# youssefg7/dl-sound-classification

Hardware: AMD Instinct MI355X
Metric: training clips/sec (EnvNet-v2, ESC-50 shape) (higher is better)
Workload: dtype bf16; 1 GPU; EnvNet-v2 train step (BC-mix, fwd, soft-CE, bwd, clip, Adam), ESC-50 shape; global_batch=256, per_gpu_batch=256, clip_samples=220500, parallelism=dp1, model=envnet_v2

## Files before the change

### dl-sound-classification_amd/csrc/common.h

```cpp
#pragma once
#include <hip/hip_runtime.h>
#include <stdint.h>
#include <stdio.h>
#include <string.h>
#include <math.h>

#include "../../include/miaudio.h"

typedef __bf16 bf16;
typedef __bf16 bf16x8 __attribute__((ext_vector_type(8)));
typedef __bf16 bf16x4 __attribute__((ext_vector_type(4)));
typedef __bf16 bf16x2 __attribute__((ext_vector_type(2)));
typedef float f32x2_cvt __attribute__((ext_vector_type(2)));
typedef unsigned u32x4 __attribute__((ext_vector_type(4)));

__device__ __forceinline__ uint32_t pk_bf16(float lo, float hi) {
  return __builtin_bit_cast(uint32_t, __builtin_convertvector(f32x2_cvt{lo, hi}, bf16x2));
}
typedef float f32x16 __attribute__((ext_vector_type(16)));
typedef float f32x4 __attribute__((ext_vector_type(4)));
typedef short s16x4 __attribute__((ext_vector_type(4)));

#define MIA_LDS __attribute__((address_space(3)))

namespace mia {
void set_error(const char* fmt, ...);
int fail(int code, const char* fmt, ...);
int cu_count();
}

#define MIA_CHECK_ARG(cond, ...)                       \
  do {                                                 \
    if (!(cond)) return mia::fail(-22, __VA_ARGS__);   \
  } while (0)

#define MIA_LAUNCH_CHECK(what)                                                   \
  do {                                                                           \
    hipError_t e__ = hipGetLastError();                                          \
    if (e__ != hipSuccess)                                                       \
      return mia::fail(-(int)e__, "%s: launch failed: %s", what, hipGetErrorString(e__)); \
  } while (0)

static inline hipStream_t as_stream(mia_stream_t s) { return reinterpret_cast<hipStream_t>(s); }
static inline int64_t cdiv(int64_t a, int64_t b) { return (a + b - 1) / b; }
static inline bool aligned16(const void* p) { return (reinterpret_cast<uintptr_t>(p) & 15) == 0; }

__device__ __forceinline__ float bf2f(bf16 x) { return (float)x; }
__device__ __forceinline__ bf16 f2bf(float x) { return (bf16)x; }

__device__ __forceinline__ void wave_sync() {
  __builtin_amdgcn_fence(__ATOMIC_ACQ_REL, "wavefront");
  __builtin_amdgcn_wave_barrier();
}

template <typename T> __device__ __forceinline__ float to_f(T x);
template <> __device__ __forceinline__ float to_f<float>(float x) { return x; }
template <> __device__ __forceinline__ float to_f<bf16>(bf16 x) { return (float)x; }
template <typename T> __device__ __forceinline__ T from_f(float x);
template <> __device__ __forceinline__ float from_f<float>(float x) { return x; }
template <> __device__ __forceinline__ bf16 from_f<bf16>(float x) { return (bf16)x; }

__device__ __forceinline__ float ld_elem(const void* p, int dtype, int64_t i) {
  return dtype == MIA_F32 ? ((const float*)p)[i] : (float)((const bf16*)p)[i];
}
__device__ __forceinline__ void st_elem(void* p, int dtype, int64_t i, float v) {
  if (dtype == MIA_F32) ((float*)p)[i] = v;
  else ((bf16*)p)[i] = (bf16)v;
}

__device__ __forceinline__ float wave_sum(float v) {
#pragma unroll
  for (int o = 32; o > 0; o >>= 1) v += __shfl_xor(v, o, 64);
  return v;
}
__device__ __forceinline__ void lds_barrier() { asm volatile("s_waitcnt lgkmcnt(0)\n\ts_barrier" ::: "memory"); }

__device__ __forceinline__ double wave_sum_d(double v) {
#pragma unroll
  for (int o = 32; o > 0; o >>= 1) v += __shfl_xor(v, o, 64);
  return v;
}
__device__ __forceinline__ double block_sum_strided(const float* __restrict__ p, int n, int64_t stride) {
  __shared__ double red_bss[256];
  double s = 0.0;
  for (int k = threadIdx.x; k < n; k += 256) s += (double)p[(int64_t)k * stride];
  red_bss[threadIdx.x] = s;
  __syncthreads();
  for (int w = 128; w > 0; w >>= 1) {
    if ((int)threadIdx.x < w) red_bss[threadIdx.x] += red_bss[threadIdx.x + w];
    __syncthreads();
  }
  const double r = red_bss[0];
  __syncthreads();
  return r;
}

constexpr int COLSUM_SLICES = 16;
inline int64_t colsum_part2_bytes(int cols) { return (int64_t)COLSUM_SLICES * cols * 8; }
static __global__ __launch_bounds__(256) void colsum_pass1_kernel(const float* __restrict__ p, int64_t rows, int cols,
                                                                  int64_t ld, double* __restrict__ part2) {
  __shared__ double red_cp[4][64];
  const int l = threadIdx.x & 63, g = threadIdx.x >> 6;
  const int c = blockIdx.x * 64 + l;
  const int64_t per = (rows + gridDim.y - 1) / gridDim.y;
  const int64_t r0 = (int64_t)blockIdx.y * per, r1 = r0 + per < rows ? r0 + per : rows;
  double s = 0.0;
  if (c < cols) {
#pragma unroll 8
    for (int64_t r = r0 + g; r < r1; r += 4) s += (double)p[r * ld + c];
  }
  red_cp[g][l] = s;
  __syncthreads();
  if (g == 0 && c < cols)
    part2[(int64_t)blockIdx.y * cols + c] = ((red_cp[0][l] + red_cp[1][l]) + red_cp[2][l]) + red_cp[3][l];
}
inline void colsum_pass1(const float* p, int64_t rows, int cols, int64_t ld, double* part2, hipStream_t s) {
  colsum_pass1_kernel<<<dim3((unsigned)((cols + 63) / 64), COLSUM_SLICES), 256, 0, s>>>(p, rows, cols, ld, part2);
}
__device__ __forceinline__ double colsum_slices(const double* __restrict__ part2, int cols, int c) {
  double v = 0.0;
#pragma unroll
  for (int y = 0; y < COLSUM_SLICES; ++y) v += part2[(int64_t)y * cols + c];
  return v;
}

__device__ __forceinline__ int mx_exponent(float amax) {
  const int be = (int)((__float_as_uint(amax) >> 23) & 0xff);
  const int e = be == 0 ? -127 : be - 127 - 8;
// ... 95 lines not shown
```

### dl-sound-classification_amd/csrc/conv3w.hip

```cpp
#include <cstdlib>

#include "bn_math.h"
#include "channel_partials.h"

namespace {

typedef unsigned u32x2 __attribute__((ext_vector_type(2)));
typedef short s16x8 __attribute__((ext_vector_type(8)));

struct W3Args {
  const bf16* x;
  const bf16* dy;
  float* part;
  int n, h, wd, oh, ow, nseg;
  const bf16* ya;
  bf16* dyo;
  float* bpart;
  const float *gamma, *scale, *shift, *mean, *invstd, *dgamma, *dbeta;
  int64_t P;
};

__device__ __forceinline__ bf16x8 tr_frag(const char* p0, int stride) {
  const s16x4 lo = __builtin_amdgcn_ds_read_tr16_b64_v4i16((MIA_LDS s16x4*)(p0));
  const s16x4 hi = __builtin_amdgcn_ds_read_tr16_b64_v4i16((MIA_LDS s16x4*)(p0 + 4 * stride));
// ... 87 lines not shown
    const int qq = lane + 64 * s;
    const int px = seg * 32 + (qq >> 2);
    const u32x4 v = {o[0], o[1], o[2], o[3]};
    *reinterpret_cast<u32x4*>(g.dyo + (((int64_t)b * g.oh + oy) * g.ow + px) * 32 + (qq & 3) * 8) = v;
    return v;
  };
  auto run = [&](const Raw& R, int it) __attribute__((always_inline)) {
    u32x4 dv[2] = {R.d[0], R.d[1]};
    if constexpr (BN) {
      dv[0] = bn_chunk(R, 0, it);
      dv[1] = bn_chunk(R, 1, it);
    }
    wave_sync();
    if (lane < 40) {
      const int l = lane;
      const int r = l / 5, q = l % 5;
      const uint32_t d[6] = {R.v[0][0], R.v[0][1], R.v[1][0], R.v[1][1], R.v[2][0], R.v[2][1]};
#pragma unroll
      for (int c = 0; c < 4; ++c) {
        uint32_t o[4];
#pragma unroll
        for (int i = 0; i < 4; ++i) {
          const int e = c + 2 * i;
          o[i] = (e & 1) ? ((d[e >> 1] >> 16) | (d[(e >> 1) + 1] << 16)) : d[e >> 1];
        }
        *reinterpret_cast<u32x4*>(sg + c * CPYB + r * ROWB + 16 * q) = u32x4{o[0], o[1], o[2], o[3]};
      }
    }
#pragma unroll
    for (int s = 0; s < 2; ++s) {
      const int qq = lane + 64 * s;
      *reinterpret_cast<u32x4*>(dt + (qq >> 2) * 64 + (qq & 3) * 16) = dv[s];
    }
    wave_sync();
    const int kx = n & 7, cp = kx & 3;
#pragma unroll
    for (int ks = 0; ks < 2; ++ks) {
      const int kr = ks * 16 + 8 * (gq >> 1) + (i16 >> 2);
      const int c4 = 16 * (gq & 1) + 4 * (i16 & 3);
      const bf16x8 fa = tr_frag(dt + kr * 64 + c4 * 2, 64);
#pragma unroll
      for (int nt = 0; nt < 2; ++nt) {
        const int ky = 4 * nt + (n >> 3);
        const char* src = sg + cp * CPYB + ky * ROWB + 2 * (16 * ks + 8 * h + (kx & 4));
        const u32x2 p0 = *reinterpret_cast<const u32x2*>(src);
        const u32x2 p1 = *reinterpret_cast<const u32x2*>(src + 8);
        const u32x4 f = {p0[0], p0[1], p1[0], p1[1]};
        acc[nt] = __builtin_amdgcn_mfma_f32_32x32x16_bf16(fa, __builtin_bit_cast(bf16x8, f), acc[nt], 0, 0, 0);
      }
    }
  };

  int it = gw;
  if (it < items) {
    Raw ra = load(it), rb;
    for (;;) {
      rb = load(it + nw);
      run(ra, it);
      it += nw;
      if (it >= items) break;
      ra = load(it + nw);
      run(rb, it);
      it += nw;
      if (it >= items) break;
    }
  }
  float* dst = g.part + (int64_t)gw * 2048;
#pragma unroll
  for (int nt = 0; nt < 2; ++nt)
#pragma unroll
    for (int r = 0; r < 16; ++r) {
      const int co = (r & 3) + 8 * (r >> 2) + 4 * h;
      dst[co * 64 + nt * 32 + n] = acc[nt][r];
    }
  if constexpr (BN) {
#pragma unroll
    for (int i = 0; i < 8; ++i)
#pragma unroll
      for (int m = 4; m < 64; m <<= 1) bs1[i] += __shfl_xor(bs1[i], m, 64);
    if (lane < 4) {
#pragma unroll
      for (int i = 0; i < 8; ++i) g.bpart[(int64_t)gw * 32 + lane * 8 + i] = bs1[i];
    }
  }
}

constexpr int C3_G = 64;
__global__ __launch_bounds__(256) void conv3_wgrad_reduce1_kernel(const float* __restrict__ part, int nslab,
                                                                  double* __restrict__ tmp) {
  const int e = blockIdx.x * 256 + threadIdx.x, gi = blockIdx.y;
  const int per = (nslab + C3_G - 1) / C3_G;
  const int w0 = gi * per, w1 = min(nslab, w0 + per);
  double s = 0.0;
  for (int w = w0; w < w1; ++w) s += (double)part[(int64_t)w * 2048 + e];
  tmp[gi * 2048 + e] = s;
}
__global__ __launch_bounds__(256) void conv3_wgrad_reduce1x16_kernel(const float* __restrict__ part, int nslab,
                                                                     double* __restrict__ tmp) {
  const int e = blockIdx.x * 256 + threadIdx.x, gi = blockIdx.y;
  const int per = (nslab + C3_G - 1) / C3_G;
  const int w0 = gi * per, w1 = min(nslab, w0 + per);
  const float* p = part + e;
  double s = 0.0;
  int w = w0;
  for (; w + 16 <= w1; w += 16) {
    float v[16];
#pragma unroll
    for (int u = 0; u < 16; ++u) v[u] = p[(int64_t)(w + u) * 2048];
#pragma unroll
    for (int u = 0; u < 16; ++u) s += (double)v[u];
  }
  for (; w < w1; ++w) s += (double)p[(int64_t)w * 2048];
  tmp[gi * 2048 + e] = s;
}
void conv3_wgrad_reduce1(const float* part, int nslab, double* tmp, hipStream_t s) {
  const char* v1 = getenv("MIA_REDUCE_V1");
  if (v1 && v1[0] == '1') conv3_wgrad_reduce1_kernel<<<dim3(8, C3_G), 256, 0, s>>>(part, nslab, tmp);
  else conv3_wgrad_reduce1x16_kernel<<<dim3(8, C3_G), 256, 0, s>>>(part, nslab, tmp);
}
__global__ __launch_bounds__(256) void conv3_wgrad_reduce2_kernel(const double* __restrict__ tmp, float* __restrict__ dw) {
  const int e = blockIdx.x * 256 + threadIdx.x;
  double s = 0.0;
#pragma unroll 8
  for (int g = 0; g < C3_G; ++g) s += tmp[g * 2048 + e];
  dw[e] = (float)s;
}

}

extern "C" int mia_conv3_wgrad(const void* x, const void* dy, float* dw, float* part, int32_t nwaves, int32_t n,
                               int32_t h, int32_t wd, mia_stream_t stream) {
  MIA_CHECK_ARG(x && dy && dw && part && n > 0 && h >= 8 && wd >= 8, "conv3_wgrad: bad arguments");
  MIA_CHECK_ARG(nwaves > 0 && nwaves % 4 == 0, "conv3_wgrad: nwaves must be a positive multiple of 4");
  MIA_CHECK_ARG(wd % 4 == 0, "conv3_wgrad: image width must be a multiple of 4 (8-byte row alignment)");
  MIA_CHECK_ARG((reinterpret_cast<uintptr_t>(dy) & 15) == 0 && (reinterpret_cast<uintptr_t>(x) & 7) == 0,
                "conv3_wgrad: dy must be 16-byte and x 8-byte aligned");
  W3Args a{reinterpret_cast<const bf16*>(x), reinterpret_cast<const bf16*>(dy), part, n, h, wd, h - 7, wd - 7,
           (int)cdiv(wd - 7, 32)};
  MIA_CHECK_ARG((int64_t)n * a.oh * a.nseg < (1ll << 31), "conv3_wgrad: too many items");
  hipStream_t s = as_stream(stream);
  conv3_wgrad_kernel<false><<<nwaves / 4, 256, 0, s>>>(a);
  MIA_LAUNCH_CHECK("conv3_wgrad");
  double* tmp = reinterpret_cast<double*>(part + (int64_t)nwaves * 2048);
  conv3_wgrad_reduce1(part, nwaves, tmp, s);
  conv3_wgrad_reduce2_kernel<<<8, 256, 0, s>>>(tmp, dw);
  MIA_LAUNCH_CHECK("conv3_wgrad_reduce");
  return 0;
}

extern "C" int64_t mia_conv3_wgrad_workspace_bytes(int32_t nwaves) {
  return (int64_t)nwaves * 2048 * 4 + (int64_t)C3_G * 2048 * 8 + (int64_t)nwaves * 32 * 4;
}

extern "C" int mia_conv3_wgrad_bn(const void* x, const void* da, const void* ya, void* dy, float* dw, float* dbias,
                                  float* part, int32_t nwaves, int32_t n, int32_t h, int32_t wd, const float* gamma,
                                  const float* scale, const float* shift, const float* mean, const float* invstd,
                                  const float* dgamma, const float* dbeta, mia_stream_t stream) {
  MIA_CHECK_ARG(x && da && ya && dy && dw && dbias && part && n > 0 && h >= 8 && wd >= 8,
                "conv3_wgrad_bn: bad arguments");
  MIA_CHECK_ARG(scale && shift && mean && invstd && dgamma && dbeta, "conv3_wgrad_bn: null BN statistics");
  MIA_CHECK_ARG(nwaves > 0 && nwaves % 4 == 0, "conv3_wgrad_bn: nwaves must be a positive multiple of 4");
  MIA_CHECK_ARG(wd % 4 == 0, "conv3_wgrad_bn: image width must be a multiple of 4 (8-byte row alignment)");
  MIA_CHECK_ARG(((reinterpret_cast<uintptr_t>(da) | reinterpret_cast<uintptr_t>(ya) | reinterpret_cast<uintptr_t>(dy)) &
                 15) == 0 && (reinterpret_cast<uintptr_t>(x) & 7) == 0,
                "conv3_wgrad_bn: da / ya / dy must be 16-byte and x 8-byte aligned");
  W3Args a{reinterpret_cast<const bf16*>(x), reinterpret_cast<const bf16*>(da), part, n, h, wd, h - 7, wd - 7,
           (int)cdiv(wd - 7, 32), reinterpret_cast<const bf16*>(ya), reinterpret_cast<bf16*>(dy), nullptr,
           gamma, scale, shift, mean, invstd, dgamma, dbeta, (int64_t)n * (h - 7) * (wd - 7)};
  MIA_CHECK_ARG((int64_t)n * a.oh * a.nseg < (1ll << 31), "conv3_wgrad_bn: too many items");
  double* tmp = reinterpret_cast<double*>(part + (int64_t)nwaves * 2048);
  a.bpart = reinterpret_cast<float*>(tmp + (int64_t)C3_G * 2048);
  hipStream_t s = as_stream(stream);
  conv3_wgrad_kernel<true><<<nwaves / 4, 256, 0, s>>>(a);
  MIA_LAUNCH_CHECK("conv3_wgrad_bn");
  conv3_wgrad_reduce1(part, nwaves, tmp, s);
  conv3_wgrad_reduce2_kernel<<<8, 256, 0, s>>>(tmp, dw);
  cp_final1_kernel<<<32, 256, 0, s>>>(a.bpart, nwaves, 32, dbias);
  MIA_LAUNCH_CHECK("conv3_wgrad_bn reduce");
  return 0;
}
```

### dl-sound-classification_amd/csrc/norm.hip

```cpp
#include "bn_math.h"
#include "channel_partials.h"

namespace {

constexpr int NT = CP_NT;

__global__ __launch_bounds__(NT) void bn_stats_kernel(const void* __restrict__ x, int dtype, int64_t P, int C,
                                                      float* __restrict__ partial) {
  const int t = threadIdx.x;
  const int G = C / 8, cg = t % G, rs = t / G, rslots = NT / G;
  float K[8];
  load8(x, dtype, (int64_t)cg * 8, K);
  float s1[8] = {0}, s2[8] = {0};
  for (int64_t r = (int64_t)blockIdx.x * rslots + rs; r < P; r += (int64_t)gridDim.x * rslots) {
    float f[8];
    load8(x, dtype, r * C + cg * 8, f);
#pragma unroll
    for (int i = 0; i < 8; ++i) {
      const float d = f[i] - K[i];
      s1[i] += d;
      s2[i] = fmaf(d, d, s2[i]);
    }
  }
  cp_fold<2>(s1, s2, C, G, rslots, blockIdx.x, partial);
}

__global__ void bn_finalize_kernel(const void* __restrict__ x, int dtype, const float* __restrict__ partial,
                                   int nblk, int64_t P, int C, const float* gamma, const float* beta,
                                   float* running_mean, float* running_var, float momentum, float eps,
                                   float* mean_o, float* invstd_o, float* scale_o, float* shift_o,
                                   const float* __restrict__ kshift = nullptr) {
  const int c = blockIdx.x;
  const double s1 = block_sum_strided(partial + (int64_t)c * 2, nblk, (int64_t)C * 2);
  const double s2 = block_sum_strided(partial + (int64_t)c * 2 + 1, nblk, (int64_t)C * 2);
  if (threadIdx.x != 0) return;
  const double n = (double)P;
  const double K = kshift ? (double)kshift[c] : (double)ld_elem(x, dtype, c);
  const double dm = s1 / n;
  const double mean = K + dm;
  double var = s2 / n - dm * dm;
  if (var < 0) var = 0;
  const float invstd = (float)(1.0 / sqrt(var + (double)eps));
  mean_o[c] = (float)mean;
  invstd_o[c] = invstd;
  const float g = gamma ? gamma[c] : 1.f, bb = beta ? beta[c] : 0.f;
  scale_o[c] = g * invstd;
  shift_o[c] = bb - (float)mean * g * invstd;
  if (running_mean) running_mean[c] = (1.f - momentum) * running_mean[c] + momentum * (float)mean;
  if (running_var) {
    const double unb = P > 1 ? var * n / (n - 1.0) : var;
    running_var[c] = (1.f - momentum) * running_var[c] + momentum * (float)unb;
  }
}

__global__ void bn_eval_kernel(int C, const float* gamma, const float* beta, const float* rm, const float* rv,
                               float eps, float* mean_o, float* invstd_o, float* scale_o, float* shift_o) {
  const int c = blockIdx.x * blockDim.x + threadIdx.x;
  if (c >= C) return;
  const float invstd = 1.f / sqrtf(rv[c] + eps);
  const float g = gamma ? gamma[c] : 1.f, bb = beta ? beta[c] : 0.f;
  mean_o[c] = rm[c];
  invstd_o[c] = invstd;
  scale_o[c] = g * invstd;
  shift_o[c] = bb - rm[c] * g * invstd;
}

__global__ __launch_bounds__(NT) void bn_relu_bwd_reduce_kernel(const void* __restrict__ dact, void* dz,
                                                                const void* __restrict__ x, int dtype, int64_t P,
                                                                int C, const float* __restrict__ scale,
                                                                const float* __restrict__ shift,
                                                                const float* __restrict__ mean,
                                                                const float* __restrict__ invstd,
                                                                float* __restrict__ partial) {
  const int t = threadIdx.x;
  const int G = C / 8, cg = t % G, rs = t / G, rslots = NT / G;
  BnRed8 bn;
  bn.load(cg, scale, shift, mean, invstd);
  float s1[8] = {0}, s2[8] = {0};
  for (int64_t r = (int64_t)blockIdx.x * rslots + rs; r < P; r += (int64_t)gridDim.x * rslots) {
    float g[8], xv[8];
    const int64_t off = r * C + cg * 8;
    load8(dact, dtype, off, g);
    load8(x, dtype, off, xv);
#pragma unroll
    for (int i = 0; i < 8; ++i) g[i] = bn.step(i, g[i], xv[i], s1[i], s2[i]);
    if (dz) store8(dz, dtype, off, g);
  }
  cp_fold<2>(s1, s2, C, G, rslots, blockIdx.x, partial);
}

template <bool MASK>
__global__ __launch_bounds__(NT) void bn_bwd_apply_kernel(const void* __restrict__ dz, const void* __restrict__ x,
                                                          void* dx, int dtype, int64_t P, int C,
                                                          const float* __restrict__ gamma,
                                                          const float* __restrict__ mean,
                                                          const float* __restrict__ invstd,
                                                          const float* __restrict__ dgamma,
                                                          const float* __restrict__ dbeta,
                                                          float* __restrict__ partial,
                                                          const float* __restrict__ scale = nullptr,
                                                          const float* __restrict__ shift = nullptr) {
  const int t = threadIdx.x;
  const int G = C / 8, cg = t % G, rs = t / G, rslots = NT / G;
  BnFwd8 m;
  if constexpr (MASK) m.load(cg, scale, shift);
  float s1[8] = {0}, s2[8] = {0};
  BnApply8 bn;
  bn.load(cg, gamma, mean, invstd, dgamma, dbeta, 1.f / (float)P);
  for (int64_t r = (int64_t)blockIdx.x * rslots + rs; r < P; r += (int64_t)gridDim.x * rslots) {
    float g[8], xv[8];
    const int64_t off = r * C + cg * 8;
    load8(dz, dtype, off, g);
    load8(x, dtype, off, xv);
#pragma unroll
    for (int i = 0; i < 8; ++i) {
      if constexpr (MASK) g[i] = bn_relu_on(xv[i], m.sc[i], m.sh[i]) ? g[i] : 0.f;
      g[i] = bn.dx(i, g[i], xv[i]);
      s1[i] += g[i];
    }
    store8(dx, dtype, off, g);
  }
  if (partial) cp_fold<2>(s1, s2, C, G, rslots, blockIdx.x, partial);
}

__global__ __launch_bounds__(NT) void colsum_kernel(const void* __restrict__ x, int dtype, int64_t P, int C,
                                                    int64_t ld, float* __restrict__ partial) {
  const int c = blockIdx.y * NT + threadIdx.x;
  if (c >= C) return;
  float s = 0.f;
  for (int64_t r = blockIdx.x; r < P; r += gridDim.x) s += ld_elem(x, dtype, r * ld + c);
  partial[(int64_t)blockIdx.x * C + c] = s;
}
__global__ __launch_bounds__(NT) void colsum8_kernel(const void* __restrict__ x, int dtype, int64_t P, int C, int64_t ld,
                                                     float* __restrict__ partial) {
  __shared__ float red[NT * 8];
  const int t = threadIdx.x;
  const int G = C / 8, Gb = G < NT ? G : NT, rslots = NT / Gb;
  const int cg = blockIdx.y * NT + t % Gb, rs = t / Gb;
  float s8[8] = {0.f, 0.f, 0.f, 0.f, 0.f, 0.f, 0.f, 0.f};
  if (rs < rslots && cg < G) {
    for (int64_t r = (int64_t)blockIdx.x * rslots + rs; r < P; r += (int64_t)gridDim.x * rslots) {
      float f[8];
      load8(x, dtype, r * ld + cg * 8, f);
#pragma unroll
      for (int i = 0; i < 8; ++i) s8[i] += f[i];
    }
  }
#pragma unroll
  for (int i = 0; i < 8; ++i) red[t * 8 + i] = s8[i];
  __syncthreads();
  for (int e = t; e < Gb * 8; e += NT) {
    const int g = e / 8, i = e % 8;
    float acc = 0.f;
    for (int r2 = 0; r2 < rslots; ++r2) acc += red[(r2 * Gb + g) * 8 + i];
    const int c = (blockIdx.y * NT + g) * 8 + i;
    if (c < C) partial[(int64_t)blockIdx.x * C + c] = acc;
  }
}

int nblocks_for(int64_t P, int C) {
  const int rslots = NT / (C / 8);
  int64_t nb = cdiv(P, (int64_t)rslots * 8);
  if (nb > CP_MAXBLK) nb = CP_MAXBLK;
  if (nb < 1) nb = 1;
  return (int)nb;
}

int check_bn(const void* x, int dtype, int64_t P, int C) {
  MIA_CHECK_ARG(x != nullptr, "bn: null input");
  MIA_CHECK_ARG(dtype == MIA_F32 || dtype == MIA_BF16, "bn: dtype");
  MIA_CHECK_ARG(C % 8 == 0 && C >= 8 && C <= 2048 && (NT % (C / 8)) == 0,
                "bn: C must be a multiple of 8 dividing 2048 (got %d)", C);
  MIA_CHECK_ARG(P > 0, "bn: empty input");
  return 0;
}

template <int PER, bool MX = false>
__global__ __launch_bounds__(NT) void ln_fwd_kernel(const void* __restrict__ x, int xdt, const float* __restrict__ g,
                                                    const float* __restrict__ b, void* y, int ydt,
                                                    float* __restrict__ mean_o, float* __restrict__ rstd_o,
                                                    int64_t rows, int D, float eps, uint8_t* __restrict__ q = nullptr,
                                                    uint8_t* __restrict__ qs = nullptr) {
  const int lane = threadIdx.x & 63;
  const int64_t row = (int64_t)blockIdx.x * 4 + (threadIdx.x >> 6);
  if (row >= rows) return;
  float v[PER];
  float s = 0.f;
#pragma unroll
  for (int i = 0; i < PER; ++i) {
    const int d = lane + 64 * i;
    v[i] = d < D ? ld_elem(x, xdt, row * D + d) : 0.f;
    s += v[i];
  }
  const float mean = wave_sum(s) / (float)D;
  float ss = 0.f;
#pragma unroll
  for (int i = 0; i < PER; ++i) {
    const int d = lane + 64 * i;
    const float dd = d < D ? v[i] - mean : 0.f;
    ss = fmaf(dd, dd, ss);
  }
  const float rstd = rsqrtf(wave_sum(ss) / (float)D + eps);
#pragma unroll
// ... 275 lines not shown
constexpr int LN_ROWS_PER_BLOCK = 256;

}

extern "C" int64_t mia_bn_partial_bytes(int64_t P, int32_t C) {
  if (C < 8 || C % 8) return 0;
  return (int64_t)CP_MAXBLK * C * 2 * 4;
}

extern "C" int mia_bn_fwd_stats(const void* x, int32_t dtype, int64_t P, int32_t C, const float* gamma,
                                const float* beta, float* running_mean, float* running_var, float momentum,
                                float eps, int32_t training, float* mean, float* invstd, float* scale,
                                float* shift, void* partial, mia_stream_t stream) {
  MIA_CHECK_ARG(mean && invstd && scale && shift, "bn_fwd_stats: null output");
  hipStream_t s = as_stream(stream);
  if (!training) {
    MIA_CHECK_ARG(running_mean && running_var, "bn_fwd_stats: eval needs running stats");
    bn_eval_kernel<<<(unsigned)cdiv(C, 256), 256, 0, s>>>(C, gamma, beta, running_mean, running_var, eps, mean, invstd,
                                                          scale, shift);
    MIA_LAUNCH_CHECK("bn_eval");
    return 0;
  }
  if (int r = check_bn(x, dtype, P, C)) return r;
  MIA_CHECK_ARG(partial != nullptr, "bn_fwd_stats: null partial workspace");
  const int nb = nblocks_for(P, C);
  bn_stats_kernel<<<nb, NT, 0, s>>>(x, dtype, P, C, (float*)partial);
  MIA_LAUNCH_CHECK("bn_stats");
  bn_finalize_kernel<<<(unsigned)C, 256, 0, s>>>(x, dtype, (const float*)partial, nb, P, C, gamma, beta,
                                                            running_mean, running_var, momentum, eps, mean, invstd,
                                                            scale, shift);
  MIA_LAUNCH_CHECK("bn_finalize");
  return 0;
}

extern "C" int mia_bn_finalize_shifted(const float* partial, int32_t nblk, int64_t P, int32_t C, const float* kshift,
                                       const float* gamma, const float* beta, float* running_mean,
                                       float* running_var, float momentum, float eps, int32_t training, float* mean,
                                       float* invstd, float* scale, float* shift, mia_stream_t stream) {
  MIA_CHECK_ARG(partial && kshift && mean && invstd && scale && shift && nblk > 0 && P > 0 && C > 0,
                "bn_finalize_shifted: bad arguments");
  MIA_CHECK_ARG(training, "bn_finalize_shifted: batch statistics are a training-mode path");
  bn_finalize_kernel<<<(unsigned)C, 256, 0, as_stream(stream)>>>(nullptr, MIA_F32, partial, nblk, P, C, gamma, beta,
                                                                running_mean, running_var, momentum, eps, mean,
                                                                invstd, scale, shift, kshift);
  MIA_LAUNCH_CHECK("bn_finalize_shifted");
  return 0;
}

extern "C" int mia_bn_relu_bwd_reduce(const void* dact, void* dz, const void* x, int32_t dtype, int64_t P,
                                      int32_t C, const float* scale, const float* shift, const float* mean,
                                      const float* invstd, float* dgamma, float* dbeta, void* partial,
                                      mia_stream_t stream) {
  if (int r = check_bn(x, dtype, P, C)) return r;
  MIA_CHECK_ARG(dact && scale && shift && mean && invstd && dgamma && dbeta && partial,
                "bn_relu_bwd_reduce: null pointer");
  hipStream_t s = as_stream(stream);
  const int nb = nblocks_for(P, C);
  bn_relu_bwd_reduce_kernel<<<nb, NT, 0, s>>>(dact, dz, x, dtype, P, C, scale, shift, mean, invstd, (float*)partial);
  MIA_LAUNCH_CHECK("bn_relu_bwd_reduce");
  cp_final2_kernel<<<(unsigned)C, 256, 0, s>>>((const float*)partial, nb, C,  dbeta,
                                                dgamma);
  MIA_LAUNCH_CHECK("channel_partial_sum");
  return 0;
}

extern "C" int mia_bn_bwd_apply(const void* dz, const void* x, void* dx, int32_t dtype, int64_t P, int32_t C,
                                const float* gamma, const float* mean, const float* invstd, const float* dgamma,
                                const float* dbeta, float* dbias, void* partial, mia_stream_t stream) {
  if (int r = check_bn(x, dtype, P, C)) return r;
  MIA_CHECK_ARG(dz && dx && mean && invstd && dgamma && dbeta, "bn_bwd_apply: null pointer");
  MIA_CHECK_ARG(!dbias || partial, "bn_bwd_apply: dbias needs the partial workspace");
  const int nb = nblocks_for(P, C);
  hipStream_t s = as_stream(stream);
  bn_bwd_apply_kernel<false><<<nb, NT, 0, s>>>(dz, x, dx, dtype, P, C, gamma, mean, invstd, dgamma, dbeta,
                                               dbias ? (float*)partial : nullptr);
  MIA_LAUNCH_CHECK("bn_bwd_apply");
  if (dbias) {
    cp_final2_kernel<<<(unsigned)C, 256, 0, s>>>((const float*)partial, nb, C,  dbias, nullptr);
    MIA_LAUNCH_CHECK("channel_partial_sum");
  }
  return 0;
}

extern "C" int mia_bn_relu_bwd_apply(const void* dact, const void* x, void* dx, int32_t dtype, int64_t P, int32_t C,
                                     const float* gamma, const float* scale, const float* shift, const float* mean,
                                     const float* invstd, const float* dgamma, const float* dbeta, float* dbias,
                                     void* partial, mia_stream_t stream) {
  if (int r = check_bn(x, dtype, P, C)) return r;
  MIA_CHECK_ARG(dact && dx && scale && shift && mean && invstd && dgamma && dbeta, "bn_relu_bwd_apply: null pointer");
  MIA_CHECK_ARG(!dbias || partial, "bn_relu_bwd_apply: dbias needs the partial workspace");
  const int nb = nblocks_for(P, C);
  hipStream_t s = as_stream(stream);
  bn_bwd_apply_kernel<true><<<nb, NT, 0, s>>>(dact, x, dx, dtype, P, C, gamma, mean, invstd, dgamma, dbeta,
                                              dbias ? (float*)partial : nullptr, scale, shift);
  MIA_LAUNCH_CHECK("bn_relu_bwd_apply");
  if (dbias) {
    cp_final2_kernel<<<(unsigned)C, 256, 0, s>>>((const float*)partial, nb, C,  dbias, nullptr);
    MIA_LAUNCH_CHECK("channel_partial_sum");
  }
  return 0;
}

extern "C" int mia_colsum(const void* x, int32_t dtype, int64_t P, int32_t C, int64_t ld, float* out, void* partial,
                          mia_stream_t stream) {
  MIA_CHECK_ARG(x && out && partial && C > 0 && P > 0 && ld >= C, "colsum: bad arguments");
  int nb = (int)std::min<int64_t>(cdiv(P, 64), MIA_COLSUM_MAXBLK);
  hipStream_t s = as_stream(stream);
  const int es = dtype == MIA_BF16 ? 2 : 4;
  if (C % 8 == 0 && ld % 8 == 0 && (reinterpret_cast<uintptr_t>(x) & 15) == 0 && (int64_t)es * 8 >= 16) {
    colsum8_kernel<<<dim3(nb, (unsigned)cdiv(C / 8, NT)), NT, 0, s>>>(x, dtype, P, C, ld, (float*)partial);
  } else {
    colsum_kernel<<<dim3(nb, (unsigned)cdiv(C, NT)), NT, 0, s>>>(x, dtype, P, C, ld, (float*)partial);
  }
  MIA_LAUNCH_CHECK("colsum");
  cp_final1_kernel<<<(unsigned)C, 256, 0, s>>>((const float*)partial, nb, C, out);
  MIA_LAUNCH_CHECK("colsum_final");
  return 0;
}

extern "C" int mia_layernorm_fwd(const void* x, int32_t xdtype, const float* gamma, const float* beta, void* y,
                                 int32_t ydtype, float* mean, float* rstd, int64_t rows, int32_t D, float eps,
                                 mia_stream_t stream) {
  MIA_CHECK_ARG(x && gamma && beta && y && mean && rstd, "layernorm_fwd: null pointer");
  MIA_CHECK_ARG(D > 0 && D <= 1024, "layernorm_fwd: D must be <= 1024");
  const unsigned nb = (unsigned)cdiv(rows, 4);
  hipStream_t s = as_stream(stream);
  const bool vec = D % 256 == 0 && (xdtype == MIA_F32 || xdtype == MIA_BF16) && (ydtype == MIA_F32 || ydtype == MIA_BF16) &&
                   ((reinterpret_cast<uintptr_t>(x) | reinterpret_cast<uintptr_t>(y) | reinterpret_cast<uintptr_t>(gamma) |
                     reinterpret_cast<uintptr_t>(beta)) & 15) == 0;
  if (vec && D == 768) ln_fwd_vec_kernel<3><<<nb, NT, 0, s>>>(x, xdtype, gamma, beta, y, ydtype, mean, rstd, rows, D, eps);
  else if (vec && D == 512) ln_fwd_vec_kernel<2><<<nb, NT, 0, s>>>(x, xdtype, gamma, beta, y, ydtype, mean, rstd, rows, D, eps);
  else if (vec && D == 256) ln_fwd_vec_kernel<1><<<nb, NT, 0, s>>>(x, xdtype, gamma, beta, y, ydtype, mean, rstd, rows, D, eps);
  else if (vec && D == 1024) ln_fwd_vec_kernel<4><<<nb, NT, 0, s>>>(x, xdtype, gamma, beta, y, ydtype, mean, rstd, rows, D, eps);
  else if (D <= 768) ln_fwd_kernel<12><<<nb, NT, 0, s>>>(x, xdtype, gamma, beta, y, ydtype, mean, rstd, rows, D, eps);
  else ln_fwd_kernel<16><<<nb, NT, 0, s>>>(x, xdtype, gamma, beta, y, ydtype, mean, rstd, rows, D, eps);
  MIA_LAUNCH_CHECK("layernorm_fwd");
  return 0;
}

extern "C" int mia_layernorm_fwd_mx(const void* x, int32_t xdtype, const float* gamma, const float* beta, void* y,
                                    void* q, void* scales, float* mean, float* rstd, int64_t rows, int32_t D, float eps,
                                    mia_stream_t stream) {
  MIA_CHECK_ARG(x && gamma && beta && y && q && scales && mean && rstd, "layernorm_fwd_mx: null pointer");
  MIA_CHECK_ARG(D > 0 && D <= 768 && D % 64 == 0, "layernorm_fwd_mx: D must be a multiple of 64, <= 768");
  const unsigned nb = (unsigned)cdiv(rows, 4);
  const bool vec = D == 768 && (xdtype == MIA_F32 || xdtype == MIA_BF16) &&
                   ((reinterpret_cast<uintptr_t>(x) | reinterpret_cast<uintptr_t>(y) | reinterpret_cast<uintptr_t>(gamma) |
                     reinterpret_cast<uintptr_t>(beta) | reinterpret_cast<uintptr_t>(q)) & 15) == 0;
  if (vec)
    ln_fwd_vec_kernel<3, true><<<nb, NT, 0, as_stream(stream)>>>(x, xdtype, gamma, beta, y, MIA_BF16, mean, rstd, rows, D,
                                                                 eps, reinterpret_cast<uint8_t*>(q),
                                                                 reinterpret_cast<uint8_t*>(scales));
  else
    ln_fwd_kernel<12, true><<<nb, NT, 0, as_stream(stream)>>>(x, xdtype, gamma, beta, y, MIA_BF16, mean, rstd, rows, D, eps,
                                                               reinterpret_cast<uint8_t*>(q), reinterpret_cast<uint8_t*>(scales));
  MIA_LAUNCH_CHECK("layernorm_fwd_mx");
  return 0;
}

static int64_t ln_rows_bytes(int64_t rows, int32_t D) {
  const int64_t a = cdiv(rows, LN_VEC_ROWS) * 3 * D * 4, b = cdiv(rows, 256) * 2 * D * 4;
  return cdiv(a > b ? a : b, 256) * 256;
}
extern "C" int64_t mia_layernorm_partial_bytes(int64_t rows, int32_t D) {
  return ln_rows_bytes(rows, D) + colsum_part2_bytes(3 * D);
}

static int layernorm_bwd_impl(const void* dy, int32_t dydtype, const void* x, int32_t xdtype, const float* gamma,
                              const float* mean, const float* rstd, void* dx, int32_t dxdtype, int32_t accumulate,
                              void* dx2, int32_t dx2dtype, float* dgamma, float* dbeta, float* dx2_colsum,
                              void* partial, int64_t rows, int32_t D, mia_stream_t stream, void* mq = nullptr,
                              void* ms = nullptr) {
  MIA_CHECK_ARG(dy && x && gamma && mean && rstd && dx && partial, "layernorm_bwd: null pointer");
  MIA_CHECK_ARG(!dx2_colsum || dx2, "layernorm_bwd: the column sums are of dx2");
  MIA_CHECK_ARG(D > 0 && D <= 1024, "layernorm_bwd: D must be <= 1024");
  hipStream_t s = as_stream(stream);
  unsigned nb;
  const bool al = ((reinterpret_cast<uintptr_t>(dy) | reinterpret_cast<uintptr_t>(x) | reinterpret_cast<uintptr_t>(dx) |
                    reinterpret_cast<uintptr_t>(dx2) | reinterpret_cast<uintptr_t>(gamma)) & 15) == 0;
  if (D == 768 && al) {
    nb = (unsigned)cdiv(rows, LN_VEC_ROWS);
    if (mq)
      ln_bwd_vec_kernel<12, true, true><<<nb, NT, 0, s>>>(dy, dydtype, x, xdtype, gamma, mean, rstd, dx, dxdtype,
// ... 58 lines not shown
```

### dl-sound-classification_amd/csrc/pool.hip

```cpp
#include <cstdlib>

#include "../../include/miaudio_pool.h"
#include "bn_math.h"
#include "channel_partials.h"

namespace {

constexpr int NT = CP_NT;

struct FastDiv {
  uint32_t d, m, l;
};
static FastDiv make_fastdiv(uint32_t d) {
  uint32_t l = 0;
  while ((1u << l) < d) ++l;
  const uint32_t m = (uint32_t)((((uint64_t)1 << 32) * (((uint64_t)1 << l) - d)) / d + 1);
  return FastDiv{d, m, l};
}
__device__ __forceinline__ uint32_t fdiv(uint32_t n, const FastDiv& f) { return (__umulhi(n, f.m) + n) >> f.l; }

__device__ __forceinline__ int64_t out_index(int layout, int b, int oy, int ox, int c, int OH, int OW, int C) {
  if (layout == 0) return (((int64_t)b * OH + oy) * OW + ox) * C + c;
  if (layout == 1) return ((int64_t)b * C + c) * OW + ox;
  return (((int64_t)b * C + c) * OH + oy) * OW + ox;
}

bool pool_v1() { const char* e = getenv("MIA_POOL_V1"); return e && e[0] == '1'; }

__device__ __forceinline__ int xcd_block_id() {
  const int nwg = gridDim.x, q = nwg / 8, r = nwg % 8, x = blockIdx.x % 8;
  return (x < r ? x * (q + 1) : r * (q + 1) + (x - r) * q) + blockIdx.x / 8;
}

template <int KH, int KW>
__device__ __forceinline__ void pool_window_dt(const void* __restrict__ x, int dtype, int64_t off0, int W, int C,
                                               int kh, int kw, const float (&sc)[8], const float (&sh)[8],
                                               float (&best)[8], float (&raw)[8], int (&arg)[8]) {
#pragma unroll
  for (int i = 0; i < 8; ++i) { best[i] = -INFINITY; raw[i] = 0.f; arg[i] = 0; }
  if constexpr (KH > 0) {
    float f[KH * KW][8];
#pragma unroll
    for (int dy = 0; dy < KH; ++dy)
#pragma unroll
      for (int dx = 0; dx < KW; ++dx) load8(x, dtype, off0 + ((int64_t)dy * W + dx) * C, f[dy * KW + dx]);
#pragma unroll
    for (int pos = 0; pos < KH * KW; ++pos)
#pragma unroll
      for (int i = 0; i < 8; ++i) {
        const float v = bn_relu(f[pos][i], sc[i], sh[i]);
        if (v > best[i]) { best[i] = v; raw[i] = f[pos][i]; arg[i] = pos; }
      }
  } else {
    for (int dy = 0; dy < kh; ++dy) {
      for (int dx = 0; dx < kw; ++dx) {
        float f[8];
        load8(x, dtype, off0 + ((int64_t)dy * W + dx) * C, f);
        const int pos = dy * kw + dx;
#pragma unroll
        for (int i = 0; i < 8; ++i) {
          const float v = bn_relu(f[i], sc[i], sh[i]);
          if (v > best[i]) { best[i] = v; raw[i] = f[i]; arg[i] = pos; }
        }
      }
    }
  }
}

template <int KH, int KW>
__device__ __forceinline__ void pool_window(const void* __restrict__ x, int dtype, int64_t off0, int W, int C, int kh,
                                            int kw, const float (&sc)[8], const float (&sh)[8], float (&best)[8],
                                            float (&raw)[8], int (&arg)[8]) {
  if (dtype == MIA_BF16) pool_window_dt<KH, KW>(x, MIA_BF16, off0, W, C, kh, kw, sc, sh, best, raw, arg);
  else if constexpr (KH * KW <= 4) pool_window_dt<KH, KW>(x, MIA_F32, off0, W, C, kh, kw, sc, sh, best, raw, arg);
  else pool_window_dt<0, 0>(x, MIA_F32, off0, W, C, kh, kw, sc, sh, best, raw, arg);
}

template <int KH, int KW>
__global__ __launch_bounds__(NT) void pool_fwd_kernel(const void* __restrict__ x, int dtype, int n, int H, int W,
                                                      int C, int kh, int kw, const float* __restrict__ scale,
                                                      const float* __restrict__ shift, void* out, int layout,
                                                      uint8_t* __restrict__ argmax, void* __restrict__ win) {
  if constexpr (KH > 0) { kh = KH; kw = KW; }
  const int OH = H / kh, OW = W / kw, G = C / 8;
  const int total = n * OH * OW * G;
  for (int idx = blockIdx.x * NT + threadIdx.x; idx < total; idx += gridDim.x * NT) {
    const int cg = idx % G;
    int p = idx / G;
    const int ox = p % OW;
    p /= OW;
    const int oy = p % OH;
    const int b = p / OH;
    BnFwd8 bn;
    float best[8], raw[8];
    int arg[8];
    bn.load_or_identity(cg, scale, shift);
    pool_window<KH, KW>(x, dtype, (((int64_t)b * H + oy * kh) * W + ox * kw) * C + cg * 8, W, C, kh, kw, bn.sc, bn.sh,
                        best, raw, arg);
    const int64_t aoff = (((int64_t)b * OH + oy) * OW + ox) * C + cg * 8;
    *reinterpret_cast<uint2*>(argmax + aoff) = argmax_pack(arg);
    if (win) store8(win, dtype, aoff, raw);
    if (layout == 0) {
// ... 454 lines not shown
#pragma unroll
        for (int i = 0; i < 8; ++i) {
          const int a = argmax_byte(am, i);
          const int iy = oy * kh + a / kw, ix = ox * kw + a % kw;
          xv[i] = ld_elem(x, dtype, (((int64_t)b * H + iy) * W + ix) * C + cg * 8 + i);
        }
      }
      float gv[8];
#pragma unroll
      for (int i = 0; i < 8; ++i) gv[i] = bn.step(i, dv[i], xv[i], s1[i], s2[i]);
      store8(gm, gdt, cell * C + cg * 8, gv);
    }
    __syncthreads();
  }
  cp_fold<2>(s1, s2, C, G, rslots, lb, partial, red);
}

template <int GDT>
__global__ __launch_bounds__(NT) void pool_bn_bwd_apply_oct_kernel(const void* __restrict__ gm,
                                                                   const uint8_t* __restrict__ argmax,
                                                                   const bf16* __restrict__ x, int n, int H, int W,
                                                                   int C, int kh, int kw, FastDiv dNO, FastDiv dH,
                                                                   FastDiv dG, const float* __restrict__ gamma,
                                                                   const float* __restrict__ mean,
                                                                   const float* __restrict__ invstd,
                                                                   const float* __restrict__ dgamma,
                                                                   const float* __restrict__ dbeta, bf16* dx,
                                                                   float* __restrict__ partial) {
  const int OH = H / kh, OW = W / kw, G = C / 8, NO = (W + 7) / 8;
  const int t = threadIdx.x;
  const int cg = t % G;
  const int P = n * H * W;
  BnApply8 bn;
  bn.load(cg, gamma, mean, invstd, dgamma, dbeta, 1.f / (float)P);
  float s1[8] = {0};
  const int64_t units = (int64_t)n * H * NO * G;
  for (int64_t u = (int64_t)blockIdx.x * NT + t; u < units; u += (int64_t)gridDim.x * NT) {
    const int rest = (int)fdiv((uint32_t)(u), dG);
    const int rowi = (int)fdiv((uint32_t)rest, dNO);
    const int o8 = rest - rowi * NO;
    const int iy = rowi - (int)fdiv((uint32_t)rowi, dH) * H;
    const int b = (rowi - iy) / H;
    const int ix0 = o8 * 8;
    const int oy = iy / kh, ox = ix0 / kw;
    const bool cell = oy < OH && ox < OW;
    const int64_t coff = cell ? (((int64_t)b * OH + oy) * OW + ox) * C + cg * 8 : 0;
    const uint2 am = *reinterpret_cast<const uint2*>(argmax + coff);
    Raw8<GDT> gr;
    gr.load(gm, coff);
    const int64_t xoff = ((int64_t)rowi * W + ix0) * C + cg * 8;
    uint4 xr[8];
#pragma unroll
    for (int j = 0; j < 8; ++j) {
      const int64_t o = ix0 + j < W ? xoff + (int64_t)j * C : xoff;
      xr[j] = *reinterpret_cast<const uint4*>(x + o);
    }
    float gv[8];
    gr.unpack(gv);
    const int pos0 = (iy - oy * kh) * kw + (ix0 - ox * kw);
#pragma unroll
    for (int j = 0; j < 8; ++j) {
      if (ix0 + j >= W) break;
      const uint32_t w4[4] = {xr[j].x, xr[j].y, xr[j].z, xr[j].w};
      uint32_t o4[4];
#pragma unroll
      for (int q = 0; q < 4; ++q) {
        float g[2];
#pragma unroll
        for (int h = 0; h < 2; ++h) {
          const int i = 2 * q + h;
          const float xv = h ? bf16_hi(w4[q]) : bf16_lo(w4[q]);
          const float gi = cell && argmax_byte(am, i) == pos0 + j ? gv[i] : 0.f;
          g[h] = bn.dx(i, gi, xv);
          s1[i] += g[h];
        }
        o4[q] = pk_bf16(g[0], g[1]);
      }
      *reinterpret_cast<uint4*>(dx + xoff + (int64_t)j * C) = uint4{o4[0], o4[1], o4[2], o4[3]};
    }
  }
  if (partial) cp_fold<1>(s1, nullptr, C, G, NT / G, blockIdx.x, partial);
}

template <int KW, int RU, int GDT>
__global__ __launch_bounds__(NT) void pool_bn_bwd_apply_run_kernel(const void* __restrict__ gm,
                                                                   const uint8_t* __restrict__ argmax,
                                                                   const bf16* __restrict__ x, int n, int H, int W,
                                                                   int C, int kh, FastDiv dNR, FastDiv dH, FastDiv dG,
                                                                   const float* __restrict__ gamma,
                                                                   const float* __restrict__ mean,
                                                                   const float* __restrict__ invstd,
                                                                   const float* __restrict__ dgamma,
                                                                   const float* __restrict__ dbeta, bf16* dx,
                                                                   float* __restrict__ partial) {
  const int OH = H / kh, OW = W / KW, G = C / 8, NR = (W + KW - 1) / KW;
  const int t = threadIdx.x;
  const int cg = t % G;
  const int P = n * H * W;
  BnApply8 bn;
  bn.load(cg, gamma, mean, invstd, dgamma, dbeta, 1.f / (float)P);
  float s1[8] = {0};
  const int units = n * H * NR * G;
  const int stride = gridDim.x * NT;
  for (int u0 = blockIdx.x * NT + t; u0 < units; u0 += RU * stride) {
    uint4 xr[RU][KW];
    uint2 am[RU];
    Raw8<GDT> gr[RU];
    int64_t xoff[RU];
    int pos0[RU], ix0[RU];
#pragma unroll
    for (int v = 0; v < RU; ++v) {
      const int u = min(u0 + v * stride, units - 1);
      const int rest = (int)fdiv((uint32_t)u, dG);
      const int rowi = (int)fdiv((uint32_t)rest, dNR);
      const int run = rest - rowi * NR;
      const int b = (int)fdiv((uint32_t)rowi, dH);
      const int iy = rowi - b * H;
      ix0[v] = run * KW;
      const int oy = iy / kh;
      const bool cell = oy < OH && run < OW;
      const int64_t coff = cell ? (((int64_t)b * OH + oy) * OW + run) * C + cg * 8 : 0;
      pos0[v] = cell ? (iy - oy * kh) * KW : -256;
      am[v] = *reinterpret_cast<const uint2*>(argmax + coff);
      gr[v].load(gm, coff);
      xoff[v] = ((int64_t)rowi * W + ix0[v]) * C + cg * 8;
#pragma unroll
      for (int j = 0; j < KW; ++j) {
        const int64_t o = ix0[v] + j < W ? xoff[v] + (int64_t)j * C : xoff[v];
        xr[v][j] = *reinterpret_cast<const uint4*>(x + o);
      }
    }
#pragma unroll
    for (int v = 0; v < RU; ++v) {
      if (u0 + v * stride >= units) break;
      float gv[8];
      gr[v].unpack(gv);
#pragma unroll
      for (int j = 0; j < KW; ++j) {
        if (ix0[v] + j >= W) break;
        const uint32_t w4[4] = {xr[v][j].x, xr[v][j].y, xr[v][j].z, xr[v][j].w};
        uint32_t o4[4];
#pragma unroll
        for (int q = 0; q < 4; ++q) {
          float g[2];
#pragma unroll
          for (int h = 0; h < 2; ++h) {
            const int i = 2 * q + h;
            const float xv = h ? bf16_hi(w4[q]) : bf16_lo(w4[q]);
            const float gi = argmax_byte(am[v], i) == pos0[v] + j ? gv[i] : 0.f;
            g[h] = bn.dx(i, gi, xv);
            s1[i] += g[h];
          }
          o4[q] = pk_bf16(g[0], g[1]);
        }
        *reinterpret_cast<uint4*>(dx + xoff[v] + (int64_t)j * C) = uint4{o4[0], o4[1], o4[2], o4[3]};
      }
    }
  }
  if (partial) cp_fold<1>(s1, nullptr, C, G, NT / G, blockIdx.x, partial);
}

#ifndef PB_UNROLL
#define PB_UNROLL 4
#endif
#ifndef PB_NB
#define PB_NB CP_MAXBLK
#endif
#ifndef PB_RUNS
#define PB_RUNS 1
#endif
template <int GDT>
__global__ __launch_bounds__(NT) void pool_bn_bwd_apply_kernel(const void* __restrict__ gm,
                                                               const uint8_t* __restrict__ argmax,
                                                               const void* __restrict__ x, int dtype, int n, int H,
                                                               int W, int C, int kh, int kw, FastDiv dW, FastDiv dH,
                                                               FastDiv dkw, FastDiv dkh,
                                                               const float* __restrict__ gamma,
                                                               const float* __restrict__ mean,
                                                               const float* __restrict__ invstd,
                                                               const float* __restrict__ dgamma,
                                                               const float* __restrict__ dbeta, void* dx,
                                                               float* __restrict__ partial) {
  const int OH = H / kh, OW = W / kw, G = C / 8;
  const int t = threadIdx.x;
  const int cg = t % G, rs = t / G, rslots = NT / G;
  const int P = n * H * W;
  float mu[8], is[8], a[8], mb[8], mg[8];
  const float invP = 1.f / (float)P;
#pragma unroll
  for (int i = 0; i < 8; ++i) {
    const int c = cg * 8 + i;
    mu[i] = mean[c]; is[i] = invstd[c];
    a[i] = (gamma ? gamma[c] : 1.f) * is[i];
    mb[i] = dbeta[c] * invP;
    mg[i] = dgamma[c] * invP;
  }
  float s1[8] = {0};
  const int stride = gridDim.x * rslots;
  for (int r0 = blockIdx.x * rslots + rs; r0 < P; r0 += PB_UNROLL * stride) {
    float xv[PB_UNROLL][8];
    uint2 am[PB_UNROLL];
    Raw8<GDT> gr[PB_UNROLL];
#pragma unroll
    for (int u = 0; u < PB_UNROLL; ++u) {
      const int r = min(r0 + u * stride, P - 1);
      load8(x, dtype, (int64_t)r * C + cg * 8, xv[u]);
      const int q = (int)fdiv(r, dW), ix = r - q * W;
      const int b = (int)fdiv(q, dH), iy = q - b * H;
      const int oy = min((int)fdiv(iy, dkh), OH - 1), ox = min((int)fdiv(ix, dkw), OW - 1);
      const int64_t coff = (((int64_t)b * OH + oy) * OW + ox) * C + cg * 8;
      am[u] = *reinterpret_cast<const uint2*>(argmax + coff);
      gr[u].load(gm, coff);
    }
#pragma unroll
    for (int u = 0; u < PB_UNROLL; ++u) {
      const int r = r0 + u * stride;
      if (r >= P) break;
      const int q = (int)fdiv(r, dW), ix = r - q * W;
      const int iy = q - (int)fdiv(q, dH) * H;
      const int oy = (int)fdiv(iy, dkh), ox = (int)fdiv(ix, dkw);
      const int pos = oy < OH && ox < OW ? (iy - oy * kh) * kw + (ix - ox * kw) : -1;
      float gv[8];
      gr[u].unpack(gv);
      float g[8];
#pragma unroll
      for (int i = 0; i < 8; ++i) {
        const uint32_t word = i < 4 ? am[u].x : am[u].y;
        const int av = (int)((word >> (8 * (i & 3))) & 0xffu);
        const float gi = av == pos ? gv[i] : 0.f;
        g[i] = a[i] * (gi - mb[i] - (xv[u][i] - mu[i]) * is[i] * mg[i]);
        s1[i] += g[i];
      }
      store8(dx, dtype, (int64_t)r * C + cg * 8, g);
    }
  }
  if (partial) cp_fold<1>(s1, nullptr, C, G, rslots, blockIdx.x, partial);
}

// ... 93 lines not shown
                "pool_bwd: null pointer");
  MIA_CHECK_ARG(c % 8 == 0 && c >= 8 && (NT % (c / 8)) == 0, "pool_bwd: channels");
  MIA_CHECK_ARG((int64_t)n * h * w < (1ll << 31), "pool_bwd: too many pixels for 32-bit indexing");
  const int rslots = NT / (c / 8);
  const int64_t P = (int64_t)n * h * w;
  hipStream_t s = as_stream(stream);
  const int nb = (int)std::max<int64_t>(1, std::min<int64_t>(cdiv(P, (int64_t)rslots * 8), CP_MAXBLK));
  pool_bwd_kernel<<<nb, NT, 0, s>>>(dout, out_layout, argmax, x, dtype, n, h, w, c, kh, kw, scale, shift, mean,
                                    invstd, dz, (float*)partial);
  MIA_LAUNCH_CHECK("pool_bwd");
  cp_final2_kernel<<<(unsigned)c, 256, 0, s>>>((const float*)partial, nb, c,  dbeta,
                                                dgamma);
  MIA_LAUNCH_CHECK("pool_bwd_final");
  return 0;
}

static int pool_grid_cap(int nb) {
  const char* e = getenv("MIA_POOL_GRID");
  const int cap = e ? atoi(e) : 0;
  return cap > 0 ? std::min(nb, cap) : nb;
}

extern "C" int mia_pool_bwd_gather_ex(const void* dout, int32_t out_layout, const uint8_t* argmax, const void* x,
                                      const void* win, int32_t dtype, int32_t n, int32_t h, int32_t w, int32_t c,
                                      int32_t kh, int32_t kw, const float* scale, const float* shift,
                                      const float* mean, const float* invstd, void* gm, int32_t gm_dtype,
                                      float* dgamma, float* dbeta, void* partial, mia_stream_t stream) {
  MIA_CHECK_ARG(dout && argmax && x && scale && shift && mean && invstd && gm && dgamma && dbeta && partial,
                "pool_bwd_gather: null pointer");
  MIA_CHECK_ARG(c % 8 == 0 && c >= 8 && (NT % (c / 8)) == 0, "pool_bwd_gather: channels");
  MIA_CHECK_ARG((int64_t)n * h * w < (1ll << 31), "pool_bwd_gather: too many pixels for 32-bit indexing");
  MIA_CHECK_ARG(h >= kh && w >= kw && kh * kw <= 256 && (reinterpret_cast<uintptr_t>(gm) & 15) == 0,
                "pool_bwd_gather: bad geometry / alignment");
  MIA_CHECK_ARG(gm_dtype == MIA_F32 || (gm_dtype == MIA_BF16 && dtype == MIA_BF16),
                "pool_bwd_gather: gm is f32, or bf16 beside bf16 activations (gm dtype %d, dtype %d)", gm_dtype, dtype);
  const int rslots = NT / (c / 8);
  const int64_t cells = (int64_t)n * (h / kh) * (w / kw);
  const int nb = pool_grid_cap((int)std::max<int64_t>(1, std::min<int64_t>(cdiv(cells, (int64_t)rslots * 2), CP_MAXBLK)));
  hipStream_t s = as_stream(stream);
  MIA_CHECK_ARG(!win || (reinterpret_cast<uintptr_t>(win) & 15) == 0, "pool_bwd_gather: win alignment");
  const bool v1 = pool_v1();
  const bool chmajor = out_layout == 2 || (out_layout == 1 && h / kh == 1);
  if (!v1 && chmajor && rslots >= 16 && cells < (1ll << 31) - 1024) {
    int lg_nch = 0;
    while ((4 << lg_nch) < rslots) ++lg_nch;
    pool_bwd_sparse_tr_kernel<<<nb, NT, 0, s>>>(dout, argmax, x, win, dtype, (int)cells, h, w, c, kh, kw, lg_nch, scale,
                                                shift, mean, invstd, gm, gm_dtype, (float*)partial);
  } else if (!v1 && win && out_layout == 0 && (dtype == MIA_BF16 || dtype == MIA_F32) &&
             (reinterpret_cast<uintptr_t>(dout) & 15) == 0 && cells + (int64_t)PG_DEPTH * nb * rslots < (1ll << 31)) {
    float* part = (float*)partial;
    const int nc = (int)cells;
    if (dtype == MIA_F32)
      pool_bwd_sparse_ra_kernel<MIA_F32, MIA_F32, PG_DEPTH><<<nb, NT, 0, s>>>(dout, win, nc, c, scale, shift, mean,
                                                                              invstd, gm, part);
    else if (gm_dtype == MIA_F32)
      pool_bwd_sparse_ra_kernel<MIA_BF16, MIA_F32, PG_DEPTH><<<nb, NT, 0, s>>>(dout, win, nc, c, scale, shift, mean,
                                                                               invstd, gm, part);
    else
      pool_bwd_sparse_ra_kernel<MIA_BF16, MIA_BF16, PG_DEPTH><<<nb, NT, 0, s>>>(dout, win, nc, c, scale, shift, mean,
                                                                                invstd, gm, part);
  } else {
    pool_bwd_sparse_kernel<<<nb, NT, 0, s>>>(dout, out_layout, argmax, x, win, dtype, n, h, w, c, kh, kw, scale, shift,
                                             mean, invstd, gm, gm_dtype, (float*)partial);
  }
  MIA_LAUNCH_CHECK("pool_bwd_gather");
  cp_final2_kernel<<<(unsigned)c, 256, 0, s>>>((const float*)partial, nb, c,  dbeta,
                                                dgamma);
  MIA_LAUNCH_CHECK("pool_bwd_gather_final");
  return 0;
}

extern "C" int mia_pool_bwd_gather(const void* dout, int32_t out_layout, const uint8_t* argmax, const void* x,
                                   const void* win, int32_t dtype, int32_t n, int32_t h, int32_t w, int32_t c, int32_t kh, int32_t kw,
                                   const float* scale, const float* shift, const float* mean, const float* invstd,
                                   float* gm, float* dgamma, float* dbeta, void* partial, mia_stream_t stream) {
  return mia_pool_bwd_gather_ex(dout, out_layout, argmax, x, win, dtype, n, h, w, c, kh, kw, scale, shift, mean, invstd,
                                gm, MIA_F32, dgamma, dbeta, partial, stream);
}

template <int GDT>
static int pool_bn_bwd_apply_launch(const void* gm, const uint8_t* argmax, const void* x, int32_t dtype, int32_t n,
                                    int32_t h, int32_t w, int32_t c, int32_t kh, int32_t kw, const float* gamma,
                                    const float* mean, const float* invstd, const float* dgamma, const float* dbeta,
                                    void* dx, float* dbias, void* partial, hipStream_t s) {
  const int rslots = NT / (c / 8);
  const int64_t P = (int64_t)n * h * w;
  const int64_t units = (int64_t)n * h * ((w + 7) / 8) * (c / 8);
  auto finish = [&](const char* what, int nb) -> int {
    MIA_LAUNCH_CHECK(what);
    if (dbias) {
      cp_final2_kernel<<<(unsigned)c, 256, 0, s>>>((const float*)partial, nb, c,  dbias, nullptr);
      MIA_LAUNCH_CHECK("pool_bn_bwd_apply_final");
    }
    return 0;
  };
  if (kw % 8 == 0 && dtype == MIA_BF16 && units < (1ll << 31) &&
      ((reinterpret_cast<uintptr_t>(x) | reinterpret_cast<uintptr_t>(dx)) & 15) == 0) {
    const int nb = (int)std::max<int64_t>(1, std::min<int64_t>(cdiv(units, NT), CP_MAXBLK));
    pool_bn_bwd_apply_oct_kernel<GDT><<<nb, NT, 0, s>>>(gm, argmax, reinterpret_cast<const bf16*>(x), n, h, w, c, kh, kw,
                                                        make_fastdiv((w + 7) / 8), make_fastdiv(h), make_fastdiv(c / 8),
                                                        gamma, mean, invstd, dgamma, dbeta, reinterpret_cast<bf16*>(dx),
                                                        dbias ? (float*)partial : nullptr);
    return finish("pool_bn_bwd_apply", nb);
  }
  const int64_t runs = (int64_t)n * h * cdiv(w, kw) * (c / 8);
  static const bool per_pixel = getenv("MIA_POOL_BWD_PIXEL") != nullptr;
  if (kw >= 2 && kw <= 4 && dtype == MIA_BF16 && runs < (1ll << 31) && !per_pixel &&
      ((reinterpret_cast<uintptr_t>(x) | reinterpret_cast<uintptr_t>(dx)) & 15) == 0) {
    constexpr int RU = PB_RUNS;
    const int nb = (int)std::max<int64_t>(1, std::min<int64_t>(cdiv(runs, (int64_t)NT * RU), PB_NB));
    const FastDiv dNR = make_fastdiv((int)cdiv(w, kw)), dH = make_fastdiv(h), dG = make_fastdiv(c / 8);
    float* part = dbias ? (float*)partial : nullptr;
    const bf16* xb = reinterpret_cast<const bf16*>(x);
    bf16* dxb = reinterpret_cast<bf16*>(dx);
    if (kw == 2)
      pool_bn_bwd_apply_run_kernel<2, RU, GDT><<<nb, NT, 0, s>>>(gm, argmax, xb, n, h, w, c, kh, dNR, dH, dG, gamma,
                                                                 mean, invstd, dgamma, dbeta, dxb, part);
    else if (kw == 3)
      pool_bn_bwd_apply_run_kernel<3, RU, GDT><<<nb, NT, 0, s>>>(gm, argmax, xb, n, h, w, c, kh, dNR, dH, dG, gamma,
                                                                 mean, invstd, dgamma, dbeta, dxb, part);
    else
      pool_bn_bwd_apply_run_kernel<4, RU, GDT><<<nb, NT, 0, s>>>(gm, argmax, xb, n, h, w, c, kh, dNR, dH, dG, gamma,
                                                                 mean, invstd, dgamma, dbeta, dxb, part);
    return finish("pool_bn_bwd_apply_run", nb);
  }
  const int nb = (int)std::max<int64_t>(1, std::min<int64_t>(cdiv(P, (int64_t)rslots * 8), CP_MAXBLK));
  pool_bn_bwd_apply_kernel<GDT><<<nb, NT, 0, s>>>(gm, argmax, x, dtype, n, h, w, c, kh, kw, make_fastdiv(w),
                                                  make_fastdiv(h), make_fastdiv(kw), make_fastdiv(kh), gamma, mean,
                                                  invstd, dgamma, dbeta, dx, dbias ? (float*)partial : nullptr);
  return finish("pool_bn_bwd_apply", nb);
}

extern "C" int mia_pool_bn_relu_bwd_apply_ex(const void* gm, int32_t gm_dtype, const uint8_t* argmax, const void* x,
                                             int32_t dtype, int32_t n, int32_t h, int32_t w, int32_t c, int32_t kh,
                                             int32_t kw, const float* gamma, const float* mean, const float* invstd,
                                             const float* dgamma, const float* dbeta, void* dx, float* dbias,
                                             void* partial, mia_stream_t stream) {
  MIA_CHECK_ARG(gm && argmax && x && mean && invstd && dgamma && dbeta && dx, "pool_bn_bwd_apply: null pointer");
  MIA_CHECK_ARG(!dbias || partial, "pool_bn_bwd_apply: dbias needs the partial workspace");
  MIA_CHECK_ARG(c % 8 == 0 && c >= 8 && (NT % (c / 8)) == 0, "pool_bn_bwd_apply: channels");
  MIA_CHECK_ARG((int64_t)n * h * w < (1ll << 31), "pool_bn_bwd_apply: too many pixels for 32-bit indexing");
  MIA_CHECK_ARG(h >= kh && w >= kw && kh * kw <= 256, "pool_bn_bwd_apply: bad geometry");
  MIA_CHECK_ARG(gm_dtype == MIA_F32 || gm_dtype == MIA_BF16, "pool_bn_bwd_apply: gm dtype %d", gm_dtype);
  MIA_CHECK_ARG((reinterpret_cast<uintptr_t>(gm) & 15) == 0, "pool_bn_bwd_apply: gm alignment");
  hipStream_t s = as_stream(stream);
  if (gm_dtype == MIA_BF16)
    return pool_bn_bwd_apply_launch<MIA_BF16>(gm, argmax, x, dtype, n, h, w, c, kh, kw, gamma, mean, invstd, dgamma,
                                              dbeta, dx, dbias, partial, s);
  return pool_bn_bwd_apply_launch<MIA_F32>(gm, argmax, x, dtype, n, h, w, c, kh, kw, gamma, mean, invstd, dgamma, dbeta,
                                           dx, dbias, partial, s);
}

extern "C" int mia_pool_bn_relu_bwd_apply(const float* gm, const uint8_t* argmax, const void* x, int32_t dtype,
                                          int32_t n, int32_t h, int32_t w, int32_t c, int32_t kh, int32_t kw,
                                          const float* gamma, const float* mean, const float* invstd,
                                          const float* dgamma, const float* dbeta, void* dx, float* dbias,
                                          void* partial, mia_stream_t stream) {
  return mia_pool_bn_relu_bwd_apply_ex(gm, MIA_F32, argmax, x, dtype, n, h, w, c, kh, kw, gamma, mean, invstd, dgamma,
                                       dbeta, dx, dbias, partial, stream);
}

extern "C" int mia_col2im_rows(const float* p, int32_t n, int32_t ph, int32_t w, int32_t kh, void* out, int32_t dtype,
                               mia_stream_t stream) {
  MIA_CHECK_ARG(p && out && n > 0 && ph > 0 && w > 0 && kh > 0, "col2im_rows: bad arguments");
  MIA_CHECK_ARG((int64_t)n * (ph + kh - 1) * w < (1ll << 31), "col2im_rows: too many elements");
  const int64_t total = (int64_t)n * (ph + kh - 1) * w;
  const int nb = (int)std::min<int64_t>(cdiv(total, 256), 16384);
  col2im_rows_kernel<<<nb, 256, 0, as_stream(stream)>>>(p, n, ph, w, kh, out, dtype);
  MIA_LAUNCH_CHECK("col2im_rows");
  return 0;
}
```

### dl-sound-classification_amd/src/miaudio/kernels.py

```python
from __future__ import annotations

import math
from dataclasses import dataclass

import os

import torch

from . import lib as L

_WS: dict = {}


def workspace(nbytes: int, device, slot: str = "main") -> torch.Tensor:
    key = (str(device), slot)
    buf = _WS.get(key)
    nbytes = max(int(nbytes), 256)
    if buf is None or buf.numel() < nbytes:
        buf = torch.empty(int(nbytes * 1.25) + 256, dtype=torch.uint8, device=device)
        _WS[key] = buf
    return buf


def _s():
# ... 208 lines not shown
            e1 = torch.cuda.Event(enable_timing=True)
            e1.record()
            PROBE[self.tag].append((self.e0, e1, self.flop, self.nbytes))
        return False


def _operand_bytes(o: L.MiaOperand, M_or_N: int, K: int) -> int:
    es = 4 if o.dtype == L.F32 else 2
    if o.kind == L.OP_DENSE:
        return o.rows * o.cols * es
    return o.n * o.h * o.w * o.c * es


def gemm(A: L.MiaOperand, B: L.MiaOperand, E: L.MiaEpilogue, M: int, N: int, K: int, compute: int,
         split_k: int | None = None, device=None, tag: str | None = None):
    lib = L.load()
    if split_k is None:
        path = lib.mia_gemm_path(A, B, M, N, K, compute, 2) if compute == L.BF16 else 0
        if path == 2:
            chunks = B.n * B.oh * -(-B.ow // 128)
            split_k = max(2, min(512, chunks // 32))
        elif path == 3:
            chunks = B.n * B.oh * -(-B.ow // 256)
            split_k = max(2, min(1024, chunks // 16))
        else:
            split_k = auto_split(M, N, K)
    ws = None
    nws = lib.mia_gemm_workspace_bytes_ex(A, B, E, M, N, K, compute, split_k)
    if nws > 0:
        ws = workspace(nws, device or torch.cuda.current_device(), "gemm")
    rec = PROBE is not None and tag in PROBE
    if rec:
        e0 = torch.cuda.Event(enable_timing=True)
        e0.record()
    L.check(lib.mia_gemm(A, B, E, M, N, K, compute, split_k, L.ptr(ws), _s()), "mia_gemm")
    if rec:
        e1 = torch.cuda.Event(enable_timing=True)
        e1.record()
        out_b = M * N * (4 if E.dtype == L.F32 else 2)
        PROBE[tag].append((e0, e1, 2 * M * N * K, _operand_bytes(A, M, K) + _operand_bytes(B, N, K) + out_b))


@dataclass
class BNState:
    mean: torch.Tensor
    invstd: torch.Tensor
    scale: torch.Tensor
    shift: torch.Tensor


def bn_fwd_stats(x: torch.Tensor, P: int, C: int, gamma, beta, running_mean, running_var, momentum: float,
                 eps: float, training: bool) -> BNState:
    dev = x.device
    st = torch.empty(4, C, dtype=torch.float32, device=dev)
    lib = L.load()
    ws = workspace(lib.mia_bn_partial_bytes(P, C), dev, "bn")
    L.check(lib.mia_bn_fwd_stats(x.data_ptr(), L.dtype_code(x), P, C, L.ptr(gamma), L.ptr(beta),
                                 L.ptr(running_mean), L.ptr(running_var), momentum, eps, int(training),
                                 st[0].data_ptr(), st[1].data_ptr(), st[2].data_ptr(), st[3].data_ptr(),
                                 ws.data_ptr(), _s()), "mia_bn_fwd_stats")
    return BNState(st[0], st[1], st[2], st[3])


def bn_relu_bwd_reduce(dact, dz, x, P, C, bn: BNState):
    dev = x.device
    g = torch.empty(2, C, dtype=torch.float32, device=dev)
    lib = L.load()
    ws = workspace(lib.mia_bn_partial_bytes(P, C), dev, "bn")
    L.check(lib.mia_bn_relu_bwd_reduce(dact.data_ptr(), L.ptr(dz), x.data_ptr(), L.dtype_code(x), P, C,
                                       bn.scale.data_ptr(), bn.shift.data_ptr(), bn.mean.data_ptr(),
                                       bn.invstd.data_ptr(), g[0].data_ptr(), g[1].data_ptr(), ws.data_ptr(),
                                       _s()), "mia_bn_relu_bwd_reduce")
    return g[0], g[1]


def bn_bwd_apply(dz, x, dx, P, C, gamma, bn: BNState, dgamma, dbeta, dbias=None):
    lib = L.load()
    ws = workspace(lib.mia_bn_partial_bytes(P, C), x.device, "bn")
    L.check(lib.mia_bn_bwd_apply(dz.data_ptr(), x.data_ptr(), dx.data_ptr(), L.dtype_code(x), P, C,
                                 L.ptr(gamma), bn.mean.data_ptr(), bn.invstd.data_ptr(), dgamma.data_ptr(),
                                 dbeta.data_ptr(), L.ptr(dbias), ws.data_ptr(), _s()), "mia_bn_bwd_apply")


def bn_relu_bwd_apply(dact, x, dx, P, C, gamma, bn: BNState, dgamma, dbeta, dbias=None):
    lib = L.load()
    ws = workspace(lib.mia_bn_partial_bytes(P, C), x.device, "bn")
    L.check(lib.mia_bn_relu_bwd_apply(dact.data_ptr(), x.data_ptr(), dx.data_ptr(), L.dtype_code(x), P, C,
                                      L.ptr(gamma), bn.scale.data_ptr(), bn.shift.data_ptr(), bn.mean.data_ptr(),
                                      bn.invstd.data_ptr(), dgamma.data_ptr(), dbeta.data_ptr(), L.ptr(dbias),
                                      ws.data_ptr(), _s()), "mia_bn_relu_bwd_apply")


def pool_bwd_gather(dout, out_layout, argmax, x, n, h, w, c, kh, kw, bn: BNState, win=None, gm_dtype=None):
    if win is not None and (win.dtype != x.dtype or win.numel() != n * (h // kh) * (w // kw) * c):
        raise ValueError("pool_bwd_gather: win must hold one x-typed value per pooled cell and channel")
    if gm_dtype is None:
        gm_dtype = torch.float32 if os.environ.get("MIA_POOL_GM32", "")[:1] == "1" else x.dtype
    dev = x.device
    g = torch.empty(2, c, dtype=torch.float32, device=dev)
    gm = torch.empty(n * (h // kh) * (w // kw), c, dtype=gm_dtype, device=dev)
    lib = L.load()
    ws = workspace(lib.mia_bn_partial_bytes(n * h * w, c), dev, "bn")
    L.check(lib.mia_pool_bwd_gather_ex(dout.data_ptr(), out_layout, argmax.data_ptr(), x.data_ptr(), L.ptr(win),
                                       L.dtype_code(x), n, h, w, c, kh, kw, bn.scale.data_ptr(), bn.shift.data_ptr(),
                                       bn.mean.data_ptr(), bn.invstd.data_ptr(), gm.data_ptr(), L.dtype_code(gm),
                                       g[0].data_ptr(), g[1].data_ptr(), ws.data_ptr(), _s()),
            "mia_pool_bwd_gather_ex")
    return gm, g[0], g[1]


def pool_bn_relu_bwd_apply(gm, argmax, x, n, h, w, c, kh, kw, gamma, bn: BNState, dgamma, dbeta, dx, dbias=None):
    lib = L.load()
    ws = workspace(lib.mia_bn_partial_bytes(n * h * w, c), x.device, "bn")
    L.check(lib.mia_pool_bn_relu_bwd_apply_ex(gm.data_ptr(), L.dtype_code(gm), argmax.data_ptr(), x.data_ptr(),
                                              L.dtype_code(x), n, h, w, c, kh, kw, L.ptr(gamma), bn.mean.data_ptr(),
                                              bn.invstd.data_ptr(), dgamma.data_ptr(), dbeta.data_ptr(),
                                              dx.data_ptr(), L.ptr(dbias), ws.data_ptr(), _s()),
            "mia_pool_bn_relu_bwd_apply_ex")


def pool_fwd(x, n, h, w, c, kh, kw, bn: BNState, out, out_layout, argmax, win=None):
    if win is not None and (win.dtype != x.dtype or win.numel() != n * (h // kh) * (w // kw) * c):
        raise ValueError("pool_fwd: win must hold one x-typed value per pooled cell and channel")
    L.check(L.load().mia_pool_fwd(x.data_ptr(), L.dtype_code(x), n, h, w, c, kh, kw, bn.scale.data_ptr(),
                                  bn.shift.data_ptr(), out.data_ptr(), out_layout, argmax.data_ptr(), L.ptr(win),
                                  _s()),
            "mia_pool_fwd")


def pool_raw_stats(x, n, h, w, c, kh, kw, gamma, kshift, win, argmax):
    assert x.dtype == torch.bfloat16 and win.dtype == torch.bfloat16 and x.is_contiguous()
    nblk = 2048
    part = torch.empty(nblk, c, 2, dtype=torch.float32, device=x.device)
    L.check(L.load().mia_pool_raw_stats(x.data_ptr(), n, h, w, c, kh, kw, gamma.data_ptr(), kshift.data_ptr(),
                                        win.data_ptr(), argmax.data_ptr(), part.data_ptr(), nblk, _s()),
            "mia_pool_raw_stats")
    return part, nblk


def pool_apply(win, n, oh, ow, c, bn: BNState, out, out_layout):
    L.check(L.load().mia_pool_apply(win.data_ptr(), n, oh, ow, c, bn.scale.data_ptr(), bn.shift.data_ptr(),
                                    out.data_ptr(), L.dtype_code(out), out_layout, _s()), "mia_pool_apply")


def pool_bwd_bn_relu_reduce(dout, out_layout, argmax, x, n, h, w, c, kh, kw, bn: BNState, dz):
    g = torch.empty(2, c, dtype=torch.float32, device=x.device)
    lib = L.load()
    ws = workspace(lib.mia_bn_partial_bytes(n * h * w, c), x.device, "bn")
    L.check(lib.mia_pool_bwd_bn_relu_reduce(dout.data_ptr(), out_layout, argmax.data_ptr(), x.data_ptr(),
                                            L.dtype_code(x), n, h, w, c, kh, kw, bn.scale.data_ptr(),
                                            bn.shift.data_ptr(), bn.mean.data_ptr(), bn.invstd.data_ptr(),
                                            dz.data_ptr(), g[0].data_ptr(), g[1].data_ptr(), ws.data_ptr(), _s()),
            "mia_pool_bwd_bn_relu_reduce")
    return g[0], g[1]


def colsum(x, P, C, ld=None):
    out = torch.empty(C, dtype=torch.float32, device=x.device)
    ws = workspace(1024 * C * 4, x.device, "colsum")
    L.check(L.load().mia_colsum(x.data_ptr(), L.dtype_code(x), P, C, C if ld is None else ld, out.data_ptr(),
                                ws.data_ptr(), _s()), "mia_colsum")
    return out


def col2im_rows(p, n, ph, w, kh, out):
    L.check(L.load().mia_col2im_rows(p.data_ptr(), n, ph, w, kh, out.data_ptr(), L.dtype_code(out), _s()),
            "mia_col2im_rows")


def conv1ch_dgrad(dy: torch.Tensor, w: torch.Tensor, n: int, oh: int, ow: int, out: torch.Tensor,
                  tag: str | None = None):
    assert dy.dtype == torch.bfloat16 and out.dtype == torch.bfloat16 and w.dtype == torch.float32
    assert dy.numel() == n * oh * ow * 32 and out.numel() == n * (oh + 7) * (ow + 7) and w.numel() == 32 * 64
    assert dy.is_contiguous() and out.is_contiguous() and w.is_contiguous()
    flop = 2.0 * n * oh * ow * 32 * 64
    with probe(tag or "", flop, dy.numel() * 2 + out.numel() * 2):
        L.check(L.load().mia_conv1ch_dgrad(dy.data_ptr(), w.data_ptr(), out.data_ptr(), n, oh, ow, _s()),
                "mia_conv1ch_dgrad")


def fe_conv1_fwd(x: torch.Tensor, w: torch.Tensor, bias: torch.Tensor, y1: torch.Tensor, n: int, t: int,
                 stats: bool, tag: str | None = None):
    w1 = (t - 64) // 2 + 1
    assert x.dtype == torch.float32 and w.dtype == torch.bfloat16 and y1.dtype == torch.bfloat16
    assert x.numel() == n * t and w.numel() == 32 * 64 and y1.numel() == n * w1 * 32 and bias.numel() == 32
    nw = 4096
    part = torch.empty(nw, 32, 2, dtype=torch.float32, device=x.device) if stats else None
    with probe(tag or "", 2.0 * n * w1 * 32 * 64, x.numel() * 4 + y1.numel() * 2):
        L.check(L.load().mia_fe_conv1_fwd(x.data_ptr(), w.data_ptr(), bias.data_ptr(), y1.data_ptr(), L.ptr(part),
                                          nw, n, t, _s()), "mia_fe_conv1_fwd")
    return (part, nw) if stats else None


def fe_conv3_fwd(x: torch.Tensor, w: torch.Tensor, bias: torch.Tensor, y: torch.Tensor, n: int, h: int, wd: int,
                 stats: bool, tag: str | None = None):
    oh, ow = h - 7, wd - 7
# ... 82 lines not shown
    return BNState(st[0], st[1], st[2], st[3])


def fe_conv2_fwd(y1: torch.Tensor, scale, shift, w: torch.Tensor, bias, y2: torch.Tensor, n: int, w1: int,
                 w2: int, tag: str | None = None):
    assert y1.dtype == torch.bfloat16 and y2.dtype == torch.bfloat16 and w.dtype == torch.bfloat16
    assert y1.numel() == n * w1 * 32 and y2.numel() == n * w2 * 64 and w.numel() == 64 * 512
    assert y1.is_contiguous() and y2.is_contiguous() and w.is_contiguous()
    flop = 2.0 * n * w2 * 64 * 512
    with probe(tag or "", flop, y1.numel() * 2 + y2.numel() * 2):
        L.check(L.load().mia_fe_conv2_fwd(y1.data_ptr(), L.ptr(scale), L.ptr(shift), w.data_ptr(), L.ptr(bias),
                                          y2.data_ptr(), n, w1, w2, _s()), "mia_fe_conv2_fwd")


def fe_conv2_dgrad(dy2: torch.Tensor, wpar: torch.Tensor, da1: torch.Tensor, n: int, w1: int, w2: int,
                   tag: str | None = None):
    assert dy2.dtype == torch.bfloat16 and da1.dtype == torch.bfloat16 and wpar.dtype == torch.bfloat16
    assert dy2.numel() == n * w2 * 64 and da1.numel() == n * w1 * 32 and wpar.numel() == 64 * 512
    assert dy2.is_contiguous() and da1.is_contiguous() and wpar.is_contiguous()
    flop = 2.0 * n * w1 * 32 * 512
    with probe(tag or "", flop, dy2.numel() * 2 + da1.numel() * 2):
        L.check(L.load().mia_fe_conv2_dgrad(dy2.data_ptr(), wpar.data_ptr(), da1.data_ptr(), n, w1, w2, _s()),
                "mia_fe_conv2_dgrad")


def fe_conv2_wgrad(dy2: torch.Tensor, y1: torch.Tensor, scale, shift, dw: torch.Tensor, n: int, w1: int, w2: int,
                   tag: str | None = None):
    assert dy2.dtype == torch.bfloat16 and y1.dtype == torch.bfloat16 and dw.dtype == torch.float32
    assert dy2.numel() == n * w2 * 64 and y1.numel() == n * w1 * 32 and dw.numel() == 64 * 512
    nlaunch = -(-(n * w1 * 64) // (2 ** 31 - 1)) + 1
    nbytes = 512 * nlaunch * 64 * 512 * 4
    ws = workspace(nbytes, dy2.device, "fw")
    flop = 2.0 * n * w2 * 64 * 512
    with probe(tag or "", flop, (dy2.numel() + y1.numel()) * 2):
        L.check(L.load().mia_fe_conv2_wgrad(dy2.data_ptr(), y1.data_ptr(), L.ptr(scale), L.ptr(shift), dw.data_ptr(),
                                            n, w1, w2, ws.data_ptr(), ws.numel(), _s()), "mia_fe_conv2_wgrad")


def fe_conv1_wgrad_bn(x: torch.Tensor, dact: torch.Tensor, y1: torch.Tensor, n: int, t: int, gamma, bn: BNState,
                      dw: torch.Tensor, dbias: torch.Tensor, tag: str | None = None):
    w1 = (t - 64) // 2 + 1
    assert dact.dtype == torch.bfloat16 and y1.dtype == torch.bfloat16 and x.dtype == torch.float32
    assert dact.numel() == n * w1 * 32 and y1.numel() == n * w1 * 32 and x.numel() == n * t
    assert dw.numel() == 32 * 64 and dw.dtype == torch.float32 and dbias.numel() == 32
    split = 512
    ws = workspace((split * (2 * 2048 + 96) + 2 * 2048 + n * 80 + 2 * 160 + 4) * 4, x.device, "tapw")
    g = torch.empty(2, 32, dtype=torch.float32, device=x.device)
    flop = 4.0 * n * w1 * 32 * 64
    with probe(tag or "", flop, (dact.numel() + y1.numel()) * 2 + x.numel() * 4):
        L.check(L.load().mia_fe_conv1_wgrad_bn(
            x.data_ptr(), dact.data_ptr(), y1.data_ptr(), n, t, bn.scale.data_ptr(), bn.shift.data_ptr(),
            L.ptr(gamma), bn.mean.data_ptr(), bn.invstd.data_ptr(), g[0].data_ptr(), g[1].data_ptr(),
            dw.data_ptr(), dbias.data_ptr(), ws.data_ptr(), split, _s()), "mia_fe_conv1_wgrad_bn")
    return g[0], g[1]


def bn_relu_apply(x: torch.Tensor, P: int, C: int, bn: BNState, out: torch.Tensor):
    assert x.dtype == torch.bfloat16 and out.dtype == torch.bfloat16 and x.numel() == P * C == out.numel()
    L.check(L.load().mia_bn_relu_apply(x.data_ptr(), P, C, bn.scale.data_ptr(), bn.shift.data_ptr(), out.data_ptr(),
                                       _s()), "mia_bn_relu_apply")


def conv_w2_fwd(x: torch.Tensor, rows: int, w: int, cin: int, wpk: torch.Tensor, bias, out: torch.Tensor,
                tag: str | None = None):
    cout = wpk.numel() // (2 * cin)
    assert x.dtype == torch.bfloat16 and wpk.dtype == torch.bfloat16 and out.dtype == torch.bfloat16
    assert x.numel() == rows * w * cin and out.numel() == rows * (w - 1) * cout
    assert x.untyped_storage().nbytes() - x.storage_offset() * 2 >= (rows * w + 1) * cin * 2, "x needs a pad pixel"
    P = rows * w
    if not W2_DROPCOPY:
        gemm(dense(x, L.KC, P, 2 * cin, ld=cin), dense(wpk, L.KC, cout, 2 * cin),
             epilogue(out, cout, bias=bias, rowmap=(w, w - 1, 1, L.RM_DROP)), P, cout, 2 * cin, L.BF16, tag=tag)
        return
    ypad = workspace(P * cout * 2, x.device, "w2fwd")[: P * cout * 2].view(torch.bfloat16)
    gemm(dense(x, L.KC, P, 2 * cin, ld=cin), dense(wpk, L.KC, cout, 2 * cin), epilogue(ypad, cout, bias=bias),
         P, cout, 2 * cin, L.BF16, tag=tag)
    L.check(L.load().mia_drop_last_col(ypad.data_ptr(), rows, w, cout, out.data_ptr(), _s()), "mia_drop_last_col")


W2_SHIFT = os.environ.get("MIA_W2_SHIFT", "0") == "1"
W2_DROPCOPY = os.environ.get("MIA_W2_DROPCOPY", "0") == "1"


def trunk_bwd_w2(dy: torch.Tensor, a: torch.Tensor, rows: int, w: int, cout: int, cin: int, wpk: torch.Tensor,
                 dw: torch.Tensor, dx: torch.Tensor, tag: str = "", wflip: torch.Tensor | None = None):
    assert dy.dtype == torch.bfloat16 and a.dtype == torch.bfloat16 and dw.dtype == torch.float32
    assert dy.numel() == rows * (w - 1) * cout and a.numel() == rows * w * cin and dw.numel() == cout * 2 * cin
    assert dx.numel() == rows * w * cin and dx.dtype == torch.bfloat16 and wpk.numel() == cout * 2 * cin
    P = rows * w
    if not W2_SHIFT and wflip is not None:
        assert a.untyped_storage().nbytes() - a.storage_offset() * 2 >= (P + 1) * cin * 2, "a needs a pad pixel"
        G = workspace((P + 1) * cout * 2, dy.device, "w2shift")[: (P + 1) * cout * 2].view(torch.bfloat16)
        L.check(L.load().mia_pad_w2(dy.data_ptr(), rows, w, cout, G.data_ptr(), a.data_ptr() + P * cin * 2, cin, _s()),
                "mia_pad_w2")
        G1 = G[cout:]
        gemm(dense(G1, L.RC, P, cout), dense(a, L.RC, P, 2 * cin, ld=cin), epilogue(dw, 2 * cin), cout, 2 * cin, P,
             L.BF16, tag=f"{tag}.wgrad" if tag else None)
        gemm(dense(G, L.KC, P, 2 * cout, ld=cout), dense(wflip, L.KC, cin, 2 * cout), epilogue(dx, cin), P, cin,
             2 * cout, L.BF16, tag=f"{tag}.dgrad" if tag else None)
        return
    ash = workspace(P * 2 * cout * 2, dy.device, "w2shift")[: P * 2 * cout * 2].view(torch.bfloat16)
    L.check(L.load().mia_shift_pad_w2(dy.data_ptr(), rows, w, cout, ash.data_ptr(), _s()), "mia_shift_pad_w2")
    gemm(dense(ash, L.RC, P, 2 * cout), dense(a, L.RC, P, cin), epilogue(dw, cin), 2 * cout, cin, P, L.BF16,
         tag=f"{tag}.wgrad" if tag else None)
    gemm(dense(ash, L.KC, P, 2 * cout), dense(wpk, L.RC, 2 * cout, cin), epilogue(dx, cin), P, cin, 2 * cout,
         L.BF16, tag=f"{tag}.dgrad" if tag else None)


def pack_weight(src: torch.Tensor, dtype: int, mode: int) -> torch.Tensor:
    cout, cin, kh, kw = src.shape
    out = torch.empty(src.numel(), dtype=L.torch_dtype(dtype), device=src.device)
    L.check(L.load().mia_pack_weight(src.data_ptr(), out.data_ptr(), dtype, cout, cin, kh, kw, mode, _s()),
            "mia_pack_weight")
    return out


def pack_weights(jobs):
    outs = []
    for s0 in range(0, len(jobs), L.PACK_BATCH):
        chunk = jobs[s0:s0 + L.PACK_BATCH]
        arr = (L.MiaPackJob * len(chunk))()
        for k, (src, dtype, mode) in enumerate(chunk):
            cout, cin, kh, kw = src.shape
            out = torch.empty(src.numel(), dtype=L.torch_dtype(dtype), device=src.device)
            arr[k] = L.MiaPackJob(src.data_ptr(), out.data_ptr(), dtype, cout, cin, kh, kw, mode)
            outs.append(out)
        L.check(L.load().mia_pack_weights(arr, len(chunk), _s()), "mia_pack_weights")
    return outs


def unpack_ohwi_grad(src_ohwi: torch.Tensor, shape, out: torch.Tensor):
    cout, cin, kh, kw = shape
    L.check(L.load().mia_pack_weight(src_ohwi.data_ptr(), out.data_ptr(), L.F32, cout, cin, kh, kw, 4, _s()),
            "mia_pack_weight(grad)")


def dropout_(x: torch.Tensor, p: float, seed: int):
    L.check(L.load().mia_dropout(x.data_ptr(), L.dtype_code(x), x.numel(), p, seed & ((1 << 64) - 1), _s()),
            "mia_dropout")


def soft_ce(logits: torch.Tensor, y: torch.Tensor, input_sigmoid: bool):
    B, C = logits.shape
    loss = torch.empty(1, dtype=torch.float32, device=logits.device)
    correct = torch.empty(1, dtype=torch.int32, device=logits.device)
    dlogits = torch.empty_like(logits)
    L.check(L.load().mia_soft_ce(logits.data_ptr(), y.data_ptr(), B, C, int(input_sigmoid), loss.data_ptr(),
                                 dlogits.data_ptr(), correct.data_ptr(), _s()), "mia_soft_ce")
    return loss[0], dlogits, correct[0]


def wait_param(p: torch.Tensor) -> None:
    ev = getattr(p, "_mia_ready", None)
    if ev is not None:
        torch.cuda.current_stream().wait_event(ev)
        p._mia_ready = None


def bf16_shadow(p: torch.Tensor) -> torch.Tensor:
    wait_param(p)
    sh = getattr(p, "_mia_bf16", None)
    if sh is not None and getattr(p, "_mia_bf16_ver", None) == p._version and sh.shape == p.shape:
        return sh
    if sh is None or sh.shape != p.shape or sh.device != p.device:
        sh = torch.empty(p.shape, dtype=torch.bfloat16, device=p.device)
    L.check(L.load().mia_cast(p.data_ptr(), L.F32, sh.data_ptr(), L.BF16, p.numel(), _s()), "mia_cast")
    p._mia_bf16 = sh
    p._mia_bf16_ver = p._version
    return sh


_SWA_TABLES: dict = {}


def _swa_table(slot: str, rows, dev) -> torch.Tensor:
    key = tuple(map(tuple, rows))
    ent = _SWA_TABLES.get((str(dev), slot))
    if ent is None or ent[0] != key:
        host = torch.tensor(rows, dtype=torch.int64).pin_memory()
        ent = _SWA_TABLES[(str(dev), slot)] = (key, host, host.to(dev, non_blocking=True))
    return ent[2]


# ... 431 lines not shown
```

### dl-sound-classification_amd/src/miaudio/lib.py

```python
from __future__ import annotations

import ctypes as C
import os
from pathlib import Path

import torch

PKG_ROOT = Path(__file__).resolve().parents[2]
LIB_PATH = Path(os.environ.get("MIAUDIO_LIB") or PKG_ROOT / "lib" / "libmiaudio.so")

F32, BF16, U8 = 0, 1, 2
MXFP8 = 16
OP_DENSE, OP_CONV, OP_CONVROW = 0, 1, 2
KC, RC = 0, 1
PRE_NONE, PRE_AFFINE, PRE_AFFINE_RELU, PRE_GELU = 0, 1, 2, 3
ACT_NONE, ACT_RELU, ACT_GELU, DACT_NZ, DACT_GELU, ACT_ADD_AUX, ACT_GELU_SAVE = 0, 1, 2, 3, 4, 5, 6
ACT_GELU_SAVE_D, DACT_MUL = 7, 8

vp = C.c_void_p
i32 = C.c_int32
i64 = C.c_int64
f32 = C.c_float


class MiaOperand(C.Structure):
    _fields_ = [("ptr", vp), ("kind", i32), ("dtype", i32), ("layout", i32), ("pre", i32),
                ("rows", i64), ("cols", i64), ("ld", i64),
                ("n", i32), ("h", i32), ("w", i32), ("c", i32),
                ("oh", i32), ("ow", i32), ("kh", i32), ("kw", i32),
                ("sh", i32), ("sw", i32), ("ph", i32), ("pw", i32),
                ("pre_scale", vp), ("pre_shift", vp)]


class MiaEpilogue(C.Structure):
    _fields_ = [("ptr", vp), ("dtype", i32), ("act", i32), ("accumulate", i32), ("aux_dtype", i32),
                ("ldc", i64), ("rm_inner", i64), ("rm_outer", i64), ("rm_istride", i64),
                ("rm_offset", i64), ("bias", vp), ("aux", vp), ("ldaux", i64),
                ("alpha", f32), ("act_scale", f32), ("sqsum", vp), ("colsum", vp), ("mx_q", vp),
                ("mx_scales", vp), ("a_colsum", vp)]


class MiaPackJob(C.Structure):
    _fields_ = [("src", vp), ("dst", vp), ("dtype", i32), ("cout", i32), ("cin", i32), ("kh", i32), ("kw", i32),
                ("mode", i32)]


PACK_BATCH = 16
RM_DROP = -1


class MiaMelCfg(C.Structure):
    _fields_ = [("sample_rate", i32), ("n_fft", i32), ("win_length", i32), ("hop", i32),
                ("n_mels", i32), ("normalize", i32), ("top_db", f32), ("target_mean", f32),
                ("target_std", f32)]


class MiaWavClip(C.Structure):
    _fields_ = [("byte_off", i64), ("frames", i64), ("channels", i32), ("format", i32)]


PCM_U8, PCM_S16, PCM_S24, PCM_S32, PCM_F32, PCM_F64 = range(6)
PCM_BYTES = (1, 2, 3, 4, 4, 8)
FIT_MODES = {"wrap": 0, "zero": 1}
WAV_MAX_CHANNELS = 8

P = C.POINTER
SIGNATURES = {
    "mia_gemm_workspace_bytes": (i64, [i64, i64, i32]),
    "mia_gemm_workspace_bytes_ex": (i64, [P(MiaOperand), P(MiaOperand), P(MiaEpilogue), i64, i64, i64, i32, i32]),
    "mia_gemm_sqsum_slots": (i64, [i64, i64]),
    "mia_gemm_sqsum_only": (C.c_int, [P(MiaOperand), P(MiaOperand), i64, i64, i64, vp, vp]),
    "mia_gemm_adam": (C.c_int, [P(MiaOperand), P(MiaOperand), i64, i64, i64, vp, vp, vp, vp, i64, vp, f32, f32, f32,
                                f32, f32, f32, vp]),
    "mia_gemm": (C.c_int, [P(MiaOperand), P(MiaOperand), P(MiaEpilogue), i64, i64, i64, i32, i32, vp, vp]),
    "mia_gemm_path": (C.c_int, [P(MiaOperand), P(MiaOperand), i64, i64, i64, i32, i32]),
    "mia_mx_quantize": (C.c_int, [vp, i32, i64, i64, i64, vp, i64, vp, vp]),
    "mia_gemm_mxfp8": (C.c_int, [vp, vp, i64, vp, vp, i64, P(MiaEpilogue), i64, i64, i64, vp]),
    "mia_mx_quantize_t": (C.c_int, [vp, i32, i64, i64, i64, vp, i64, vp, vp]),
    "mia_gemm_mxfp8_workspace_bytes": (i64, [i64, i64, i32]),
    "mia_gemm_mxfp8_ex": (C.c_int, [vp, vp, i64, vp, vp, i64, P(MiaEpilogue), i64, i64, i64, vp, vp]),
    "mia_layernorm_fwd_mx": (C.c_int, [vp, i32, vp, vp, vp, vp, vp, vp, vp, i64, i32, f32, vp]),
    "mia_attn_fwd_mx": (C.c_int, [vp, vp, vp, vp, vp, i32, i32, i32, f32, vp]),
    "mia_splitk_reduce": (C.c_int, [vp, i32, i64, i64, P(MiaEpilogue), vp]),
    "mia_logmel_workspace_bytes": (i64, [i64, i64]),
    "mia_logmel_fwd": (C.c_int, [vp, i64, i64, i64, P(MiaMelCfg), vp, vp, vp, vp, vp, vp, vp, vp, vp, vp, vp]),
    "mia_bn_partial_bytes": (i64, [i64, i32]),
    "mia_bn_fwd_stats": (C.c_int, [vp, i32, i64, i32, vp, vp, vp, vp, f32, f32, i32, vp, vp, vp, vp, vp, vp]),
    "mia_bn_relu_bwd_reduce": (C.c_int, [vp, vp, vp, i32, i64, i32, vp, vp, vp, vp, vp, vp, vp, vp]),
    "mia_bn_bwd_apply": (C.c_int, [vp, vp, vp, i32, i64, i32, vp, vp, vp, vp, vp, vp, vp, vp]),
    "mia_bn_relu_bwd_apply": (C.c_int, [vp, vp, vp, i32, i64, i32, vp, vp, vp, vp, vp, vp, vp, vp, vp, vp]),
    "mia_pool_bwd_gather": (C.c_int, [vp, i32, vp, vp, vp, i32, i32, i32, i32, i32, i32, i32, vp, vp, vp, vp, vp, vp,
                                      vp, vp, vp]),
    "mia_pool_bn_relu_bwd_apply": (C.c_int, [vp, vp, vp, i32, i32, i32, i32, i32, i32, i32, vp, vp, vp, vp, vp, vp,
                                             vp, vp, vp]),
    "mia_pool_bwd_gather_ex": (C.c_int, [vp, i32, vp, vp, vp, i32, i32, i32, i32, i32, i32, i32, vp, vp, vp, vp, vp,
                                         i32, vp, vp, vp, vp]),
    "mia_pool_bn_relu_bwd_apply_ex": (C.c_int, [vp, i32, vp, vp, i32, i32, i32, i32, i32, i32, i32, vp, vp, vp, vp, vp,
                                                vp, vp, vp, vp]),
    "mia_pool_fwd": (C.c_int, [vp, i32, i32, i32, i32, i32, i32, i32, vp, vp, vp, i32, vp, vp, vp]),
    "mia_pool_bwd_bn_relu_reduce": (C.c_int, [vp, i32, vp, vp, i32, i32, i32, i32, i32, i32, i32, vp, vp, vp,
                                              vp, vp, vp, vp, vp, vp]),
    "mia_colsum": (C.c_int, [vp, i32, i64, i32, i64, vp, vp, vp]),
    "mia_col2im_rows": (C.c_int, [vp, i32, i32, i32, i32, vp, i32, vp]),
    "mia_conv1ch_dgrad": (C.c_int, [vp, vp, vp, i32, i32, i32, vp]),
    "mia_fe_conv2_fwd": (C.c_int, [vp, vp, vp, vp, vp, vp, i32, i32, i32, vp]),
    "mia_fe_conv2_dgrad": (C.c_int, [vp, vp, vp, i32, i32, i32, vp]),
    "mia_bn_relu_apply": (C.c_int, [vp, i64, i32, vp, vp, vp, vp]),
    "mia_shift_pad_w2": (C.c_int, [vp, i64, i32, i32, vp, vp]),
    "mia_pad_w2": (C.c_int, [vp, i64, i32, i32, vp, vp, i32, vp]),
    "mia_drop_last_col": (C.c_int, [vp, i64, i32, i32, vp, vp]),
    "mia_fe_conv1_fwd": (C.c_int, [vp, vp, vp, vp, vp, i32, i32, i32, vp]),
    "mia_fe_conv3_fwd": (C.c_int, [vp, vp, vp, vp, vp, i32, i32, i32, i32, vp]),
    "mia_pool_raw_stats": (C.c_int, [vp, i32, i32, i32, i32, i32, i32, vp, vp, vp, vp, vp, i32, vp]),
    "mia_pool_apply": (C.c_int, [vp, i32, i32, i32, i32, vp, vp, vp, i32, i32, vp]),
    "mia_conv3_wgrad": (C.c_int, [vp, vp, vp, vp, i32, i32, i32, i32, vp]),
    "mia_conv3_wgrad_workspace_bytes": (C.c_int64, [i32]),
    "mia_conv3_wgrad_bn": (C.c_int, [vp, vp, vp, vp, vp, vp, vp, i32, i32, i32, i32, vp, vp, vp, vp, vp, vp, vp, vp]),
    "mia_trunk_conv8": (C.c_int, [vp, vp, vp, vp, vp, vp, vp, i32, i32, i32, i32, i32, i32, vp]),
    "mia_trunk_conv8_dgrad_bn": (C.c_int, [vp, vp, vp, i32, i32, i32, i32, vp, vp, vp, vp, vp, vp, vp, vp, vp]),
    "mia_bn_finalize_shifted": (C.c_int, [vp, i32, i64, i32, vp, vp, vp, vp, vp, C.c_float, C.c_float, i32, vp, vp, vp,
                                          vp, vp]),
    "mia_fe_conv2_wgrad": (C.c_int, [vp, vp, vp, vp, vp, i32, i32, i32, vp, i64, vp]),
    "mia_fe_conv1_wgrad_bn": (C.c_int, [vp, vp, vp, i32, i32, vp, vp, vp, vp, vp, vp, vp, vp, vp, vp, i32, vp]),
    "mia_pack_weight": (C.c_int, [vp, vp, i32, i32, i32, i32, i32, i32, vp]),
    "mia_pack_weights": (C.c_int, [P(MiaPackJob), i32, vp]),
    "mia_dropout": (C.c_int, [vp, i32, i64, f32, C.c_uint64, vp]),
    "mia_soft_ce": (C.c_int, [vp, vp, i32, i32, i32, vp, vp, vp, vp]),
    "mia_adam_workspace_bytes": (i64, [i32]),
    "mia_adam_coef_offset": (i64, [i32]),
    "mia_clip_adam": (C.c_int, [vp, vp, vp, vp, vp, vp, i32, i64, i64, f32, f32, f32, f32, f32, i32, f32, vp, vp, vp, vp,
                                vp, vp]),
    "mia_layernorm_fwd": (C.c_int, [vp, i32, vp, vp, vp, i32, vp, vp, i64, i32, f32, vp]),
    "mia_layernorm_bwd": (C.c_int, [vp, i32, vp, i32, vp, vp, vp, vp, i32, i32, vp, i32, vp, vp, vp, i64, i32, vp]),
    "mia_layernorm_partial_bytes": (i64, [i64, i32]),
    "mia_layernorm_bwd_colsum": (C.c_int, [vp, i32, vp, i32, vp, vp, vp, vp, i32, i32, vp, i32, vp, vp, vp, vp, i64,
                                           i32, vp]),
    "mia_layernorm_bwd_colsum_mx": (C.c_int, [vp, i32, vp, i32, vp, vp, vp, vp, i32, i32, vp, vp, vp, vp, vp, vp, vp, i64, i32, vp]),
    "mia_attn_fwd": (C.c_int, [vp, vp, vp, i32, i32, i32, i32, f32, vp]),
    "mia_attn_bwd": (C.c_int, [vp, vp, vp, vp, vp, vp, i32, i32, i32, i32, f32, vp]),
    "mia_attn_bwd_workspace_bytes": (C.c_int64, [i32, i32, i32, i32]),
    "mia_attn_saved_q_bytes": (C.c_int64, [i32, i32, i32]),
    "mia_attn_bwd_chain_bytes": (C.c_int64, [i32, i32, i32]),
    "mia_attn_bwd_onepass": (C.c_int, [vp, vp, vp, vp, vp, vp, vp, vp, i32, i32, i32, f32, i32, vp]),
    "mia_attn_fwd_save_q": (C.c_int, [vp, vp, vp, vp, vp, vp, i32, i32, i32, f32, vp]),
    "mia_attn_bwd_saved_q": (C.c_int, [vp, vp, vp, vp, vp, vp, i32, i32, i32, f32, vp]),
    "mia_attn_bwd_two_pass": (C.c_int, [vp, vp, vp, vp, vp, vp, i32, i32, i32, f32, i32, vp]),
    "mia_attn_bwd_fused": (C.c_int, [vp, vp, vp, vp, vp, vp, i32, i32, i32, f32, i32, vp]),
    "mia_attn_bwd_error_offset": (C.c_int64, [i32, i32, i32]),
    "mia_attn_fwd_dropout": (C.c_int, [vp, vp, vp, vp, i32, i32, i32, i32, f32, f32, C.c_uint64, vp]),
    "mia_attn_bwd_dropout": (C.c_int, [vp, vp, vp, vp, vp, vp, i32, i32, i32, i32, f32, f32, C.c_uint64, i32, vp]),
    "mia_dropout_apply": (C.c_int, [vp, i32, vp, vp, i32, i64, f32, C.c_uint64, vp]),
    "mia_stream_copy": (C.c_int, [vp, vp, i64, vp]),
    "mia_mfma_rate_sink_floats": (i64, [i32]),
    "mia_mfma_rate": (C.c_int, [vp, i32, i32, vp]),
    "mia_tokens_fwd": (C.c_int, [vp, vp, vp, vp, i32, i32, i32, vp]),
    "mia_tokens_bwd": (C.c_int, [vp, vp, vp, vp, i32, i32, i32, vp]),
    "mia_ast_patches": (C.c_int, [vp, i32, i32, i32, i32, i32, vp, vp]),
    "mia_tokens_fwd_inplace": (C.c_int, [vp, vp, vp, i32, i32, i32, vp]),
    "mia_cast": (C.c_int, [vp, i32, vp, i32, i64, vp]),
    "mia_add_inplace": (C.c_int, [vp, vp, i32, i64, vp]),
    "mia_bc_mix": (C.c_int, [vp, vp, i64, i32, vp, vp, vp, vp, i32, vp, vp, vp, vp, vp]),
    "mia_bc_partner": (C.c_int, [vp, i32, vp, i32, vp, vp, vp]),
    "mia_stretch_gain": (C.c_int, [vp, i64, i32, vp, vp, vp, vp]),
    "mia_spec_augment_mixup":(C.c_int, [vp, vp, vp, i32, i32, i32, vp, vp, vp, vp, vp, vp, vp]),
    "mia_leaf_workspace_bytes": (i64, [i32, i64, i32, i32, i32, i32]),
    "mia_leaf_energy_fwd": (C.c_int, [vp, vp, vp, i32, i64, i32, i32, i32, i32, vp, vp]),
    "mia_leaf_energy_bwd": (C.c_int, [vp, vp, vp, vp, i32, i64, i32, i32, i32, i32, vp, vp]),
    "mia_pcen_workspace_bytes": (i64, [i32, i32]),
    "mia_pcen_fwd": (C.c_int, [vp, vp, vp, f32, vp, i32, i32, i32, vp]),
    "mia_pcen_bwd": (C.c_int, [vp, vp, vp, f32, vp, vp, vp, vp, vp, i32, i32, i32, vp]),
    "mia_lt_stats_blocks": (i32, [i32, i32, i32, i32]),
    "mia_lt_workspace_bytes": (i64, [i32]),
    "mia_lt_pool_stats": (C.c_int, [vp, i32, i32, i32, i32, i32, vp, vp, vp, vp, vp, i32, vp]),
    "mia_lt_pool_apply": (C.c_int, [vp, i32, i32, i32, i32, vp, vp, vp, i32, i32, vp]),
    "mia_lt_pool_bwd_gather": (C.c_int, [vp, i32, i32, vp, i32, i32, i32, i32, vp, vp, vp, vp, vp, vp, vp, vp, vp]),
    "mia_lt_pool_bwd_apply": (C.c_int, [vp, vp, vp, i32, i32, i32, i32, i32, vp, vp, vp, vp, vp, vp, vp, vp, vp]),
    "mia_lt_pcen_fwd": (C.c_int, [vp, vp, vp, f32, vp, i32, i32, i32, i32, i32, vp]),
    "mia_lt_pcen_bwd": (C.c_int, [vp, vp, vp, f32, vp, i32, vp, vp, vp, vp, i32, i32, i32, i32, vp]),
    "mia_resample_out_len": (i64, [i64, i32, i32]),
    "mia_resample": (C.c_int, [vp, i64, i32, i64, vp, vp, i32, i32, i32, vp, i64, i64, vp]),
    "mia_clip_sgd": (C.c_int, [vp, vp, vp, vp, vp, i32, i64, i64, f32, f32, f32, f32, i32, f32, vp, vp, vp, vp, vp,
# ... 84 lines not shown
```

### dl-sound-classification_amd/src/models/envnet_hip.py

```python
from __future__ import annotations

import itertools
import os

import torch

from ..miaudio import kernels as K
from ..miaudio import lib as L
from .bn_cma import update_factor

_SEED = itertools.count(0x5EED)
C8_BNSEP = os.environ.get("MIA_C8_BNSEP", "0") == "1"
C3_BNSEP = os.environ.get("MIA_C3_BNSEP", "0") == "1"
FC1_CHUNK_ROWS = 256


def _use_conv8(cd: int, cin: int, cout: int, kh: int, kw: int) -> bool:
    return cd == L.BF16 and cin == 32 and cout == 32 and kh == 8 and kw == 8

TRUNK = [
    (("trunk", 0, 0), ("trunk", 0, 1), 1, 32, 8, 8),
    (("trunk", 0, 3), ("trunk", 0, 4), 32, 32, 8, 8),
    (("trunk", 1, 0), ("trunk", 1, 1), 32, 64, 1, 4),
    (("trunk", 1, 3), ("trunk", 1, 4), 64, 64, 1, 4),
# ... 227 lines not shown
    def backward(ctx, glogits):
        s = ctx.saved
        p = ctx.params
        g = s["g"]
        B, cd = s["B"], s["cd"]
        tdt = L.torch_dtype(cd)
        dev = glogits.device
        bns = _bns(ctx.model)
        grads = [None] * len(p)
        glogits = glogits.contiguous().float()
        keep_scale = 1.0 / (1.0 - s["drop_p"]) if s["drop_p"] > 0 else 1.0
        ready = getattr(ctx.model, "_grad_ready", None)
        chunk_ready = getattr(ctx.model, "_grad_chunk_ready", None)
        gather = getattr(ctx.model, "_grad_gather", None)

        def emit(lo, hi):
            if ready is None:
                return
            ready([(p[i], grads[i]) for i in range(lo, hi)])
            for i in range(lo, hi):
                grads[i] = None

        acts = [s["flat"], s["h1"], s["h2"]]
        dcur = glogits
        for li in (2, 1, 0):
            Wt = s["wfc"][li]
            fout, fin = Wt.shape
            hin = acts[li]
            dW = torch.empty(fout, fin, dtype=torch.float32, device=dev) if li > 0 else None
            if (li == 0 and gather is not None and cd == L.BF16 and fout % 128 == 0 and fin % 128 == 0
                    and B % 64 == 0 and gather(p[40], dcur, hin)):
                pass
            elif li == 0 and chunk_ready is not None and fout % FC1_CHUNK_ROWS == 0 and fout > FC1_CHUNK_ROWS:
                dW = torch.empty(fout, fin, dtype=torch.float32, device=dev)
                for lo in range(0, fout, FC1_CHUNK_ROWS):
                    part = dW[lo:lo + FC1_CHUNK_ROWS]
                    K.gemm(K.dense(dcur[:, lo:], L.RC, B, FC1_CHUNK_ROWS, ld=fout), K.dense(hin, L.RC, B, fin),
                           K.epilogue(part, fin), FC1_CHUNK_ROWS, fin, B, cd, tag="fc1.wgrad")
                    chunk_ready(p[40], dW, part, lo + FC1_CHUNK_ROWS == fout)
            elif (li == 0 and ready is None and chunk_ready is None and cd == L.BF16 and p[40].grad is None
                  and K.defers_to_fused_adam(p[40]) and fout % 128 == 0 and fin % 128 == 0
                  and B % 64 == 0):
                K.defer_weight_grad(p[40], K.dense(dcur, L.RC, B, fout), K.dense(hin, L.RC, B, fin), fout, fin, B,
                                    keep=(dcur, hin), tag="fc1.wgrad")
            else:
                if dW is None:
                    dW = torch.empty(fout, fin, dtype=torch.float32, device=dev)
                sq = K.sqsum_slots(dW, fout, fin) if li < 2 else None
                K.gemm(K.dense(dcur, L.RC, B, fout), K.dense(hin, L.RC, B, fin), K.epilogue(dW, fin, sqsum=sq), fout,
                       fin, B, cd, tag=f"fc{li + 1}.wgrad")
                if sq is not None:
                    K.tag_sqsum(p[40 + 2 * li], dW, sq)
            grads[40 + 2 * li] = dW
            grads[41 + 2 * li] = K.colsum(dcur, B, fout)
            if li > 0:
                dprev = torch.empty(B, fin, dtype=tdt, device=dev)
                K.gemm(K.dense(dcur, L.KC, B, fout), K.dense(Wt, L.RC, fout, fin),
                       K.epilogue(dprev, fin, act=L.DACT_NZ, aux=hin, ldaux=fin, act_scale=keep_scale),
                       B, fin, fout, cd, tag=f"fc{li + 1}.dgrad")
            else:
                dprev = torch.empty(B, fin, dtype=tdt, device=dev)
                K.gemm(K.dense(dcur, L.KC, B, fout), K.dense(Wt, L.RC, fout, fin), K.epilogue(dprev, fin),
                       B, fin, fout, cd, tag=f"fc{li + 1}.dgrad")
            dcur = dprev
            emit(40 + 2 * li, 42 + 2 * li)

        wpk = s["wpk"]
        bjobs = [(8 + 8 * b + o, 1) for b in range(4) for o in (0, 4)] + [(4, 2)]
        bjobs += [(8 + 8 * b, 3) for b in range(4) if TRUNK[2 * b][2] == 1]
        wbk = dict(zip(bjobs, K.pack_weights([(p[i], cd, m) for i, m in bjobs])))
        dpool = dcur
        for blk in (3, 2, 1, 0):
            ts = s["trunk"][blk]
            (H, W), (ha, wa), (hb, wb), (hp, wp) = g["trunk"][blk]
            _, _, cin, cout, kh, kw = TRUNK[2 * blk]
            _, _, cin2, cout2, kh2, kw2 = TRUNK[2 * blk + 1]
            pa = 8 + 8 * blk
            ph, pw = TRUNK_POOL[blk]
            Pb = B * hb * wb
            lay = 2 if blk == 3 else 0
            gm, dgb, dbb = K.pool_bwd_gather(dpool, lay, ts["am"], ts["yb"], B, hb, wb, cout2, ph, pw, ts["bnb"],
                                             win=ts["win"])
            grads[pa + 6], grads[pa + 7] = dgb, dbb
            dyb = torch.empty(Pb, cout2, dtype=tdt, device=dev)
            dbias_b = torch.empty(cout2, dtype=torch.float32, device=dev)
            K.pool_bn_relu_bwd_apply(gm, ts["am"], ts["yb"], B, hb, wb, cout2, ph, pw, bns[3 + 2 * blk].weight,
                                     ts["bnb"], dgb, dbb, dyb, dbias_b)
            grads[pa + 5] = dbias_b
            Kb = kh2 * kw2 * cin2
            dWb = torch.empty(cout2, Kb, dtype=torch.float32, device=dev)
            Pa = B * ha * wa
            da = torch.empty(Pa, cout, dtype=tdt, device=dev)
            red = None
            if ts["act"] is not None:
                K.trunk_bwd_w2(dyb, ts["act"], B * ha, wa, cout2, cin2, wpk[pa + 4], dWb, da, wflip=wbk[(pa + 4, 1)],
                               tag=f"t{blk}b")
            else:
                K.gemm(K.dense(dyb, L.RC, Pb, cout2),
                       K.conv(ts["ya"], L.RC, B, ha, wa, cin2, hb, wb, kh2, kw2, pre=L.PRE_AFFINE_RELU,
                              scale=ts["bna"].scale, shift=ts["bna"].shift),
                       K.epilogue(dWb, Kb), cout2, Kb, Pb, cd, tag=f"t{blk}b.wgrad")
                wbf = wbk[(pa + 4, 1)]
                Kdb = kh2 * kw2 * cout2
                if _use_conv8(cd, cin2, cout2, kh2, kw2) and not C8_BNSEP:
                    red = K.trunk_conv8_dgrad_bn(dyb, wbf, da, B, hb, wb, ts["ya"], ts["bna"], tag=f"t{blk}b.dgrad")
                elif _use_conv8(cd, cin2, cout2, kh2, kw2):
                    K.trunk_conv8(dyb, wbf, da, B, hb, wb, ph=kh2 - 1, pw=kw2 - 1, tag=f"t{blk}b.dgrad")
                else:
                    K.gemm(K.conv(dyb, L.KC, B, hb, wb, cout2, ha, wa, kh2, kw2, ph=kh2 - 1, pw=kw2 - 1),
                           K.dense(wbf, L.KC, cin2, Kdb), K.epilogue(da, cin2), Pa, cin2, Kdb, cd,
                           tag=f"t{blk}b.dgrad")
            gwb = torch.empty_like(p[pa + 4])
            K.unpack_ohwi_grad(dWb, p[pa + 4].shape, gwb)
            grads[pa + 4] = gwb
            dga, dba = red if red is not None else K.bn_relu_bwd_reduce(da, None, ts["ya"], Pa, cout, ts["bna"])
            grads[pa + 2], grads[pa + 3] = dga, dba
            dbias_a = torch.empty(cout, dtype=torch.float32, device=dev)
            grads[pa + 1] = dbias_a
            dya = da
            Ka = kh * kw * cin
            dWa = torch.empty(cout, Ka, dtype=torch.float32, device=dev)
            dense_w2 = ts["act"] is not None
            c3w = cin == 1 and cd == L.BF16 and kh == 8 and kw == 8 and cout == 32 and W % 4 == 0
            if c3w and not C3_BNSEP:
                K.conv3_wgrad_bn(ts["inp"], da, ts["ya"], da, dWa, dbias_a, B, H, W, bns[2 + 2 * blk].weight,
                                 ts["bna"], dga, dba, tag=f"t{blk}a.wgrad")
            else:
                K.bn_relu_bwd_apply(da, ts["ya"], da, Pa, cout, bns[2 + 2 * blk].weight, ts["bna"], dga, dba,
                                    dbias_a)
            if c3w and not C3_BNSEP:
                pass
            elif dense_w2:
                dinp = torch.empty(B * H * W, cin, dtype=tdt, device=dev)
                K.trunk_bwd_w2(dya, ts["inp"].reshape(B * H * W, cin), B * H, W, cout, cin, wpk[pa],
                               dWa, dinp, tag=f"t{blk}a", wflip=wbk[(pa, 1)])
            elif c3w:
                K.conv3_wgrad(ts["inp"], dya, dWa, B, H, W, tag=f"t{blk}a.wgrad")
            else:
                if cin == 1:
                    Bop = K.conv(ts["inp"], L.RC, B, H, W, 1, ha, wa, kh, kw, row_kind=True)
                else:
                    Bop = K.conv(ts["inp"], L.RC, B, H, W, cin, ha, wa, kh, kw)
                K.gemm(K.dense(dya, L.RC, Pa, cout), Bop, K.epilogue(dWa, Ka), cout, Ka, Pa, cd,
                       tag=f"t{blk}a.wgrad")
            gwa = torch.empty_like(p[pa])
            K.unpack_ohwi_grad(dWa, p[pa].shape, gwa)
            grads[pa] = gwa
            if dense_w2:
                pass
            elif cin == 1 and cd == L.BF16 and kh == 8 and kw == 8 and cout == 32:
                dinp = torch.empty(B, H, W, dtype=tdt, device=dev)
                K.conv1ch_dgrad(dya, p[pa], B, ha, wa, dinp, tag=f"t{blk}a.dgrad")
            elif cin == 1:
                wr = wbk[(pa, 3)]
                Pm = torch.empty(B * ha * W, kh, dtype=torch.float32, device=dev)
                K.gemm(K.conv(dya, L.KC, B, ha, wa, cout, ha, W, 1, kw, pw=kw - 1),
                       K.dense(wr, L.KC, kh, kw * cout), K.epilogue(Pm, kh), B * ha * W, kh, kw * cout, cd,
                       tag=f"t{blk}a.dgrad")
                dinp = torch.empty(B, H, W, dtype=tdt, device=dev)
                K.col2im_rows(Pm, B, ha, W, kh, dinp)
            else:
                waf = wbk[(pa, 1)]
                dinp = torch.empty(B * H * W, cin, dtype=tdt, device=dev)
                Kda = kh * kw * cout
                K.gemm(K.conv(dya, L.KC, B, ha, wa, cout, H, W, kh, kw, ph=kh - 1, pw=kw - 1),
                       K.dense(waf, L.KC, cin, Kda), K.epilogue(dinp, cin), B * H * W, cin, Kda, cd,
                       tag=f"t{blk}a.dgrad")
            dpool = dinp
            emit(pa, pa + 8)

        fe = K.probe("frontend.bwd", *_frontend_work(B, g, tdt, backward=True))
        fe.__enter__()
        W1, W2, Wp = g["W1"], g["W2"], g["Wp"]
        P2, P1 = B * W2, B * W1
        gm, dg2, db2 = K.pool_bwd_gather(dpool, 1, s["am0"], s["y2"], B, 1, W2, 64, 1, 64, s["bn2"], win=s["win0"])
        grads[6], grads[7] = dg2, db2
        dy2 = torch.empty(P2, 64, dtype=tdt, device=dev)
        dbias2 = torch.empty(64, dtype=torch.float32, device=dev)
        K.pool_bn_relu_bwd_apply(gm, s["am0"], s["y2"], B, 1, W2, 64, 1, 64, bns[1].weight, s["bn2"], dg2, db2, dy2,
                                 dbias2)
        grads[5] = dbias2
        dW2 = torch.empty(64, 512, dtype=torch.float32, device=dev)
        if cd == L.BF16:
            K.fe_conv2_wgrad(dy2, s["y1"], s["bn1"].scale, s["bn1"].shift, dW2, B, W1, W2, tag="conv2.wgrad")
        else:
            K.gemm(K.dense(dy2, L.RC, P2, 64),
                   K.conv(s["y1"], L.RC, B, 1, W1, 32, 1, W2, 1, 16, sw=2, pre=L.PRE_AFFINE_RELU,
                          scale=s["bn1"].scale, shift=s["bn1"].shift),
                   K.epilogue(dW2, 512), 64, 512, P2, cd, tag="conv2.wgrad")
        gw2 = torch.empty_like(p[4])
        K.unpack_ohwi_grad(dW2, p[4].shape, gw2)
        grads[4] = gw2
        wpar = wbk[(4, 2)]
        da1 = torch.empty(P1, 32, dtype=tdt, device=dev)
        if cd == L.BF16:
            K.fe_conv2_dgrad(dy2, wpar, da1, B, W1, W2, tag="conv2.dgrad")
        else:
            wpar = wpar.view(2, 32 * 8 * 64)
            for par in (0, 1):
                Tp = (W1 - par + 1) // 2
                K.gemm(K.conv(dy2, L.KC, B, 1, W2, 64, 1, Tp, 1, 8, pw=7),
                       K.dense(wpar[par], L.KC, 32, 512),
                       K.epilogue(da1, 32, rowmap=(Tp, W1, 2, par)), B * Tp, 32, 512, cd, tag="conv2.dgrad")
        dbias1 = torch.empty(32, dtype=torch.float32, device=dev)
        dW1 = torch.empty(32, 64, dtype=torch.float32, device=dev)
        T = g["T"]
        if cd == L.BF16:
            dg1, db1 = K.fe_conv1_wgrad_bn(s["x"], da1, s["y1"], B, T, bns[0].weight, s["bn1"], dW1, dbias1,
                                           tag="conv1.wgrad")
            grads[2], grads[3] = dg1, db1
        else:
            dg1, db1 = K.bn_relu_bwd_reduce(da1, None, s["y1"], P1, 32, s["bn1"])
            grads[2], grads[3] = dg1, db1
            K.bn_relu_bwd_apply(da1, s["y1"], da1, P1, 32, bns[0].weight, s["bn1"], dg1, db1, dbias1)
            K.gemm(K.dense(da1, L.RC, P1, 32), K.conv(s["x"], L.RC, B, 1, T // 2, 2, 1, W1, 1, 32, row_kind=True),
                   K.epilogue(dW1, 64), 32, 64, P1, cd, tag="conv1.wgrad")
        grads[1] = dbias1
        grads[0] = dW1.view_as(p[0])
# ... 9 lines not shown
```

Measured before the change: 16260 clips/s.

## Write BN-ReLU backward outputs directly in padded w2 layout and pipeline conv3 wgrad

The BN-ReLU backward apply kernels (plain and pool variants) gain a row-map mode. It writes gradients straight into the shifted and padded buffer that the width-2 trunk backward GEMMs consume, zeroing the pad pixels, so the separate mia_pad_w2 pass and its extra round trip through memory go away. A new conv3 wgrad+BN kernel becomes the default. It software-pipelines global loads three items deep, uses incremental position stepping instead of per-item divisions, and keeps BN constants in registers. Env knobs allow a grid cap and fallback to the old kernel. This adds more code paths and register pressure.

```diff
diff --git a/dl-sound-classification_amd/csrc/common.h b/dl-sound-classification_amd/csrc/common.h
--- a/dl-sound-classification_amd/csrc/common.h
+++ b/dl-sound-classification_amd/csrc/common.h
@@ -44,6 +44,23 @@
 static inline hipStream_t as_stream(mia_stream_t s) { return reinterpret_cast<hipStream_t>(s); }
 static inline int64_t cdiv(int64_t a, int64_t b) { return (a + b - 1) / b; }
 static inline bool aligned16(const void* p) { return (reinterpret_cast<uintptr_t>(p) & 15) == 0; }
+
+struct FastDiv {
+  uint32_t d, m, l;
+};
+static inline FastDiv make_fastdiv(uint32_t d) {
+  uint32_t l = 0;
+  while ((1u << l) < d) ++l;
+  const uint32_t m = (uint32_t)((((uint64_t)1 << 32) * (((uint64_t)1 << l) - d)) / d + 1);
+  return FastDiv{d, m, l};
+}
+__device__ __forceinline__ uint32_t fdiv(uint32_t n, const FastDiv& f) { return (__umulhi(n, f.m) + n) >> f.l; }
+
+struct RowMap {
+  int lead, rowpx;
+  void* zp;
+  int zc16;
+};
 
 __device__ __forceinline__ float bf2f(bf16 x) { return (float)x; }
 __device__ __forceinline__ bf16 f2bf(float x) { return (bf16)x; }
diff --git a/dl-sound-classification_amd/csrc/conv3w.hip b/dl-sound-classification_amd/csrc/conv3w.hip
--- a/dl-sound-classification_amd/csrc/conv3w.hip
+++ b/dl-sound-classification_amd/csrc/conv3w.hip
@@ -193,6 +193,203 @@
 #pragma unroll
       for (int i = 0; i < 8; ++i) g.bpart[(int64_t)gw * 32 + lane * 8 + i] = bs1[i];
     }
+  }
+}
+
+struct W3Step { int dseg, doy, db; };
+struct W3Pos { int seg, oy, b; };
+
+template <bool BNREG>
+__global__ __launch_bounds__(256) void conv3_wgrad_bn2_kernel(W3Args g, W3Step st) {
+  constexpr int ROWB = 80, CPYB = 704;
+  __shared__ __attribute__((aligned(16))) char strip[4][4 * CPYB];
+  __shared__ __attribute__((aligned(16))) char dyt[4][32 * 64];
+  __shared__ __attribute__((aligned(16))) float bnp[7][32];
+  const int lane = threadIdx.x & 63, wv = __builtin_amdgcn_readfirstlane(threadIdx.x >> 6);
+  const int gw = blockIdx.x * 4 + wv, nw = gridDim.x * 4;
+  const int items = g.n * g.oh * g.nseg;
+  char* sg = strip[wv];
+  char* dt = dyt[wv];
+  f32x16 acc[2];
+#pragma unroll
+  for (int i = 0; i < 16; ++i) { acc[0][i] = 0.f; acc[1][i] = 0.f; }
+  struct Raw { u32x2 v[3]; u32x4 d[2]; u32x4 y[2]; uint32_t ok; };
+  float bs1[8];
+  if (threadIdx.x < 32) {
+    const int c = threadIdx.x;
+    const float invP = 1.f / (float)g.P;
+    const float is = g.invstd[c];
+    bnp[0][c] = g.scale[c];
+    bnp[1][c] = g.shift[c];
+    bnp[2][c] = (g.gamma ? g.gamma[c] : 1.f) * is;
+    bnp[3][c] = g.mean[c];
+    bnp[4][c] = is;
+    bnp[5][c] = g.dbeta[c] * invP;
+    bnp[6][c] = g.dgamma[c] * invP;
+  }
+#pragma unroll
+  for (int i = 0; i < 8; ++i) bs1[i] = 0.f;
+  __syncthreads();
+  float creg[BNREG ? 7 : 1][8];
+  if constexpr (BNREG) {
+#pragma unroll
+    for (int k = 0; k < 7; ++k)
+#pragma unroll
+      for (int i = 0; i < 8; ++i) creg[k][i] = bnp[k][(lane & 3) * 8 + i];
+  }
+  auto cst = [&](int k, int i) __attribute__((always_inline)) -> float {
+    if constexpr (BNREG) return creg[k][i];
+    else return bnp[k][(lane & 3) * 8 + i];
+  };
+  auto next = [&](const W3Pos& p, int idx) __attribute__((always_inline)) -> W3Pos {
+    if (idx >= items) return p;
+    W3Pos q = p;
+    q.seg += st.dseg;
+    const int c0 = q.seg >= g.nseg ? 1 : 0;
+    q.seg -= c0 ? g.nseg : 0;
+    q.oy += st.doy + c0;
+    const int c1 = q.oy >= g.oh ? 1 : 0;
+    q.oy -= c1 ? g.oh : 0;
+    q.b += st.db + c1;
+    return q;
+  };
+  auto load = [&](const W3Pos& p) __attribute__((always_inline)) {
+    Raw R;
+    const int l = lane < 40 ? lane : lane - 40;
+    const int r = l / 5, q = l % 5;
+    const int col = p.seg * 32 + 8 * q;
+    const bf16* src = g.x + ((int64_t)p.b * g.h + p.oy + r) * g.wd;
+#pragma unroll
+    for (int k = 0; k < 3; ++k) {
+      const int c = col + 4 * k;
+      R.v[k] = c + 4 <= g.wd ? *reinterpret_cast<const u32x2*>(src + c) : u32x2{0u, 0u};
+    }
+    const int64_t drow = ((int64_t)p.b * g.oh + p.oy) * g.ow * 32;
+    R.ok = 0;
+#pragma unroll
+    for (int s = 0; s < 2; ++s) {
+      const int qq = lane + 64 * s;
+      const int px = p.seg * 32 + (qq >> 2);
+      const int64_t off = drow + (int64_t)px * 32 + (qq & 3) * 8;
+      R.d[s] = px < g.ow ? *reinterpret_cast<const u32x4*>(g.dy + off) : u32x4{0u, 0u, 0u, 0u};
+      R.y[s] = px < g.ow ? *reinterpret_cast<const u32x4*>(g.ya + off) : u32x4{0u, 0u, 0u, 0u};
+      R.ok |= (uint32_t)(px < g.ow) << s;
+    }
+    return R;
+  };
+  const int i16 = lane & 15, gq = lane >> 4, h = lane >> 5;
+  const int n = lane & 31;
+  auto bn_chunk = [&](const Raw& R, int s, const W3Pos& p) __attribute__((always_inline)) -> u32x4 {
+    if (!((R.ok >> s) & 1u)) return u32x4{0u, 0u, 0u, 0u};
+    uint32_t o[4];
+#pragma unroll
+    for (int k = 0; k < 4; ++k) {
+      const uint32_t dw = R.d[s][k], yw = R.y[s][k];
+      float gv[2] = {bf16_lo(dw), bf16_hi(dw)};
+      const float xv[2] = {bf16_lo(yw), bf16_hi(yw)};
+#pragma unroll
+      for (int j = 0; j < 2; ++j) {
+        const int i = 2 * k + j;
+        gv[j] = bn_relu_on(xv[j], cst(0, i), cst(1, i)) ? gv[j] : 0.f;
+        gv[j] = bn_dx(gv[j], xv[j], cst(2, i), cst(3, i), cst(4, i), cst(5, i), cst(6, i));
+        bs1[i] += gv[j];
+      }
+      o[k] = pk_bf16(gv[0], gv[1]);
+    }
+    const int qq = lane + 64 * s;
+    const int px = p.seg * 32 + (qq >> 2);
+    const u32x4 v = {o[0], o[1], o[2], o[3]};
+    *reinterpret_cast<u32x4*>(g.dyo + (((int64_t)p.b * g.oh + p.oy) * g.ow + px) * 32 + (qq & 3) * 8) = v;
+    return v;
+  };
+  auto run = [&](const Raw& R, const W3Pos& p) __attribute__((always_inline)) {
+    u32x4 dv[2];
+    dv[0] = bn_chunk(R, 0, p);
+    dv[1] = bn_chunk(R, 1, p);
+    wave_sync();
+    if (lane < 40) {
+      const int l = lane;
+      const int r = l / 5, q = l % 5;
+      const uint32_t d[6] = {R.v[0][0], R.v[0][1], R.v[1][0], R.v[1][1], R.v[2][0], R.v[2][1]};
+#pragma unroll
+      for (int c = 0; c < 4; ++c) {
+        uint32_t o[4];
+#pragma unroll
+        for (int i = 0; i < 4; ++i) {
+          const int e = c + 2 * i;
+          o[i] = (e & 1) ? ((d[e >> 1] >> 16) | (d[(e >> 1) + 1] << 16)) : d[e >> 1];
+        }
+        *reinterpret_cast<u32x4*>(sg + c * CPYB + r * ROWB + 16 * q) = u32x4{o[0], o[1], o[2], o[3]};
+      }
+    }
+#pragma unroll
+    for (int s = 0; s < 2; ++s) {
+      const int qq = lane + 64 * s;
+      *reinterpret_cast<u32x4*>(dt + (qq >> 2) * 64 + (qq & 3) * 16) = dv[s];
+    }
+    wave_sync();
+    const int kx = n & 7, cp = kx & 3;
+#pragma unroll
+    for (int ks = 0; ks < 2; ++ks) {
+      const int kr = ks * 16 + 8 * (gq >> 1) + (i16 >> 2);
+      const int c4 = 16 * (gq & 1) + 4 * (i16 & 3);
+      const bf16x8 fa = tr_frag(dt + kr * 64 + c4 * 2, 64);
+#pragma unroll
+      for (int nt = 0; nt < 2; ++nt) {
+        const int ky = 4 * nt + (n >> 3);
+        const char* src = sg + cp * CPYB + ky * ROWB + 2 * (16 * ks + 8 * h + (kx & 4));
+        const u32x2 p0 = *reinterpret_cast<const u32x2*>(src);
+        const u32x2 p1 = *reinterpret_cast<const u32x2*>(src + 8);
+        const u32x4 f = {p0[0], p0[1], p1[0], p1[1]};
+        acc[nt] = __builtin_amdgcn_mfma_f32_32x32x16_bf16(fa, __builtin_bit_cast(bf16x8, f), acc[nt], 0, 0, 0);
+      }
+    }
+  };
+
+  int it = gw;
+  if (it < items) {
+    W3Pos p0;
+    {
+      const int rest = it / g.nseg;
+      p0.seg = it - rest * g.nseg;
+      p0.b = rest / g.oh;
+      p0.oy = rest - p0.b * g.oh;
+    }
+    W3Pos p1 = next(p0, it + nw), p2 = next(p1, it + 2 * nw);
+    Raw r0 = load(p0), r1 = load(p1), r2;
+    for (;;) {
+      r2 = load(p2);
+      run(r0, p0);
+      it += nw;
+      if (it >= items) break;
+      p0 = next(p2, it + 2 * nw);
+      r0 = load(p0);
+      run(r1, p1);
+      it += nw;
+      if (it >= items) break;
+      p1 = next(p0, it + 2 * nw);
+      r1 = load(p1);
+      run(r2, p2);
+      it += nw;
+      if (it >= items) break;
+      p2 = next(p1, it + 2 * nw);
+    }
+  }
+  float* dst = g.part + (int64_t)gw * 2048;
+#pragma unroll
+  for (int nt = 0; nt < 2; ++nt)
+#pragma unroll
+    for (int r = 0; r < 16; ++r) {
+      const int co = (r & 3) + 8 * (r >> 2) + 4 * h;
+      dst[co * 64 + nt * 32 + n] = acc[nt][r];
+    }
+#pragma unroll
+  for (int i = 0; i < 8; ++i)
+#pragma unroll
+    for (int m = 4; m < 64; m <<= 1) bs1[i] += __shfl_xor(bs1[i], m, 64);
+  if (lane < 4) {
+#pragma unroll
+    for (int i = 0; i < 8; ++i) g.bpart[(int64_t)gw * 32 + lane * 8 + i] = bs1[i];
   }
 }
 
@@ -282,7 +479,20 @@
   double* tmp = reinterpret_cast<double*>(part + (int64_t)nwaves * 2048);
   a.bpart = reinterpret_cast<float*>(tmp + (int64_t)C3_G * 2048);
   hipStream_t s = as_stream(stream);
-  conv3_wgrad_kernel<true><<<nwaves / 4, 256, 0, s>>>(a);
+  const char* e = getenv("MIA_C3W_GRID");
+  const int cap = e ? atoi(e) : 0;
+  const int nblk = cap > 0 ? std::min(nwaves / 4, cap) : nwaves / 4;
+  nwaves = nblk * 4;
+  const char* v1 = getenv("MIA_C3W_V1");
+  const char* lds = getenv("MIA_C3W_BNLDS");
+  if (v1 && v1[0] == '1') {
+    conv3_wgrad_kernel<true><<<nblk, 256, 0, s>>>(a);
+  } else {
+    const int t = nwaves / a.nseg;
+    const W3Step st{nwaves % a.nseg, t % a.oh, t / a.oh};
+    if (lds && lds[0] == '1') conv3_wgrad_bn2_kernel<false><<<nblk, 256, 0, s>>>(a, st);
+    else conv3_wgrad_bn2_kernel<true><<<nblk, 256, 0, s>>>(a, st);
+  }
   MIA_LAUNCH_CHECK("conv3_wgrad_bn");
   conv3_wgrad_reduce1(part, nwaves, tmp, s);
   conv3_wgrad_reduce2_kernel<<<8, 256, 0, s>>>(tmp, dw);
diff --git a/dl-sound-classification_amd/csrc/norm.hip b/dl-sound-classification_amd/csrc/norm.hip
--- a/dl-sound-classification_amd/csrc/norm.hip
+++ b/dl-sound-classification_amd/csrc/norm.hip
@@ -1,3 +1,4 @@
+#include "../../include/miaudio_rowmap.h"
 #include "bn_math.h"
 #include "channel_partials.h"
 
@@ -89,7 +90,7 @@
   cp_fold<2>(s1, s2, C, G, rslots, blockIdx.x, partial);
 }
 
-template <bool MASK>
+template <bool MASK, bool RM = false>
 __global__ __launch_bounds__(NT) void bn_bwd_apply_kernel(const void* __restrict__ dz, const void* __restrict__ x,
                                                           void* dx, int dtype, int64_t P, int C,
                                                           const float* __restrict__ gamma,
@@ -99,7 +100,8 @@
                                                           const float* __restrict__ dbeta,
                                                           float* __restrict__ partial,
                                                           const float* __restrict__ scale = nullptr,
-                                                          const float* __restrict__ shift = nullptr) {
+                                                          const float* __restrict__ shift = nullptr,
+                                                          RowMap rm = RowMap{}, int w = 0, FastDiv dW = FastDiv{}) {
   const int t = threadIdx.x;
   const int G = C / 8, cg = t % G, rs = t / G, rslots = NT / G;
   BnFwd8 m;
@@ -107,6 +109,10 @@
   float s1[8] = {0}, s2[8] = {0};
   BnApply8 bn;
   bn.load(cg, gamma, mean, invstd, dgamma, dbeta, 1.f / (float)P);
+  if constexpr (RM) {
+    if (rm.zp && blockIdx.x == 0)
+      for (int i = t; i < rm.zc16; i += NT) reinterpret_cast<uint4*>(rm.zp)[i] = uint4{0u, 0u, 0u, 0u};
+  }
   for (int64_t r = (int64_t)blockIdx.x * rslots + rs; r < P; r += (int64_t)gridDim.x * rslots) {
     float g[8], xv[8];
     const int64_t off = r * C + cg * 8;
@@ -118,7 +124,18 @@
       g[i] = bn.dx(i, g[i], xv[i]);
       s1[i] += g[i];
     }
-    store8(dx, dtype, off, g);
+    if constexpr (RM) {
+      const int row = (int)fdiv((uint32_t)r, dW), ix = (int)r - row * w;
+      const int64_t pix = rm.lead + (int64_t)row * rm.rowpx + ix;
+      store8(dx, dtype, pix * C + cg * 8, g);
+      const float z[8] = {0.f, 0.f, 0.f, 0.f, 0.f, 0.f, 0.f, 0.f};
+      if (ix == w - 1)
+        for (int px = 1; px <= rm.rowpx - w; ++px) store8(dx, dtype, (pix + px) * C + cg * 8, z);
+      if (r == 0)
+        for (int px = 0; px < rm.lead; ++px) store8(dx, dtype, (int64_t)px * C + cg * 8, z);
+    } else {
+      store8(dx, dtype, off, g);
+    }
   }
   if (partial) cp_fold<2>(s1, s2, C, G, rslots, blockIdx.x, partial);
 }
@@ -560,23 +577,44 @@
   return 0;
 }
 
+extern "C" int mia_bn_relu_bwd_apply_rows(const void* dact, const void* x, void* dx, int32_t dtype, int64_t P,
+                                          int32_t C, int32_t w, int32_t lead, int32_t row_pixels, void* zero_pixel,
+                                          int32_t zc, const float* gamma, const float* scale, const float* shift,
+                                          const float* mean, const float* invstd, const float* dgamma,
+                                          const float* dbeta, float* dbias, void* partial, mia_stream_t stream) {
+  if (int r = check_bn(x, dtype, P, C)) return r;
+  MIA_CHECK_ARG(dact && dx && scale && shift && mean && invstd && dgamma && dbeta, "bn_relu_bwd_apply: null pointer");
+  MIA_CHECK_ARG(!dbias || partial, "bn_relu_bwd_apply: dbias needs the partial workspace");
+  MIA_CHECK_ARG(w > 0 && P % w == 0 && lead >= 0 && row_pixels >= w && zc >= 0 && zc % 8 == 0 && (zc == 0 || zero_pixel),
+                "bn_relu_bwd_apply: bad row map (w %d, lead %d, row_pixels %d, zc %d)", w, lead, row_pixels, zc);
+  const int nb = nblocks_for(P, C);
+  hipStream_t s = as_stream(stream);
+  if (lead != 0 || row_pixels != w || zc) {
+    MIA_CHECK_ARG(P < (1ll << 31) && dx != dact, "bn_relu_bwd_apply: a row map needs P < 2^31 and dx apart from dact");
+    MIA_CHECK_ARG(aligned16(dx) && (!zc || aligned16(zero_pixel)), "bn_relu_bwd_apply: dx / zero_pixel alignment");
+    const int es = dtype == MIA_BF16 ? 2 : 4;
+    const RowMap rm{lead, row_pixels, zc ? zero_pixel : nullptr, zc * es / 16};
+    bn_bwd_apply_kernel<true, true><<<nb, NT, 0, s>>>(dact, x, dx, dtype, P, C, gamma, mean, invstd, dgamma, dbeta,
+                                                      dbias ? (float*)partial : nullptr, scale, shift, rm, w,
+                                                      make_fastdiv((uint32_t)w));
+  } else {
+    bn_bwd_apply_kernel<true><<<nb, NT, 0, s>>>(dact, x, dx, dtype, P, C, gamma, mean, invstd, dgamma, dbeta,
+                                                dbias ? (float*)partial : nullptr, scale, shift);
+  }
+  MIA_LAUNCH_CHECK("bn_relu_bwd_apply");
+  if (dbias) {
+    cp_final2_kernel<<<(unsigned)C, 256, 0, s>>>((const float*)partial, nb, C,  dbias, nullptr);
+    MIA_LAUNCH_CHECK("channel_partial_sum");
+  }
+  return 0;
+}
+
 extern "C" int mia_bn_relu_bwd_apply(const void* dact, const void* x, void* dx, int32_t dtype, int64_t P, int32_t C,
                                      const float* gamma, const float* scale, const float* shift, const float* mean,
                                      const float* invstd, const float* dgamma, const float* dbeta, float* dbias,
                                      void* partial, mia_stream_t stream) {
-  if (int r = check_bn(x, dtype, P, C)) return r;
-  MIA_CHECK_ARG(dact && dx && scale && shift && mean && invstd && dgamma && dbeta, "bn_relu_bwd_apply: null pointer");
-  MIA_CHECK_ARG(!dbias || partial, "bn_relu_bwd_apply: dbias needs the partial workspace");
-  const int nb = nblocks_for(P, C);
-  hipStream_t s = as_stream(stream);
-  bn_bwd_apply_kernel<true><<<nb, NT, 0, s>>>(dact, x, dx, dtype, P, C, gamma, mean, invstd, dgamma, dbeta,
-                                              dbias ? (float*)partial : nullptr, scale, shift);
-  MIA_LAUNCH_CHECK("bn_relu_bwd_apply");
-  if (dbias) {
-    cp_final2_kernel<<<(unsigned)C, 256, 0, s>>>((const float*)partial, nb, C,  dbias, nullptr);
-    MIA_LAUNCH_CHECK("channel_partial_sum");
-  }
-  return 0;
+  return mia_bn_relu_bwd_apply_rows(dact, x, dx, dtype, P, C, 1, 0, 1, nullptr, 0, gamma, scale, shift, mean, invstd,
+                                    dgamma, dbeta, dbias, partial, stream);
 }
 
 extern "C" int mia_colsum(const void* x, int32_t dtype, int64_t P, int32_t C, int64_t ld, float* out, void* partial,
diff --git a/dl-sound-classification_amd/csrc/pool.hip b/dl-sound-classification_amd/csrc/pool.hip
--- a/dl-sound-classification_amd/csrc/pool.hip
+++ b/dl-sound-classification_amd/csrc/pool.hip
@@ -1,23 +1,13 @@
 #include <cstdlib>
 
 #include "../../include/miaudio_pool.h"
+#include "../../include/miaudio_rowmap.h"
 #include "bn_math.h"
 #include "channel_partials.h"
 
 namespace {
 
 constexpr int NT = CP_NT;
-
-struct FastDiv {
-  uint32_t d, m, l;
-};
-static FastDiv make_fastdiv(uint32_t d) {
-  uint32_t l = 0;
-  while ((1u << l) < d) ++l;
-  const uint32_t m = (uint32_t)((((uint64_t)1 << 32) * (((uint64_t)1 << l) - d)) / d + 1);
-  return FastDiv{d, m, l};
-}
-__device__ __forceinline__ uint32_t fdiv(uint32_t n, const FastDiv& f) { return (__umulhi(n, f.m) + n) >> f.l; }
 
 __device__ __forceinline__ int64_t out_index(int layout, int b, int oy, int ox, int c, int OH, int OW, int C) {
   if (layout == 0) return (((int64_t)b * OH + oy) * OW + ox) * C + c;
@@ -638,7 +628,7 @@
   if (partial) cp_fold<1>(s1, nullptr, C, G, NT / G, blockIdx.x, partial);
 }
 
-template <int KW, int RU, int GDT>
+template <int KW, int RU, int GDT, bool RM = false>
 __global__ __launch_bounds__(NT) void pool_bn_bwd_apply_run_kernel(const void* __restrict__ gm,
                                                                    const uint8_t* __restrict__ argmax,
                                                                    const bf16* __restrict__ x, int n, int H, int W,
@@ -648,11 +638,15 @@
                                                                    const float* __restrict__ invstd,
                                                                    const float* __restrict__ dgamma,
                                                                    const float* __restrict__ dbeta, bf16* dx,
-                                                                   float* __restrict__ partial) {
+                                                                   float* __restrict__ partial, RowMap rm = RowMap{}) {
   const int OH = H / kh, OW = W / KW, G = C / 8, NR = (W + KW - 1) / KW;
   const int t = threadIdx.x;
   const int cg = t % G;
   const int P = n * H * W;
+  if constexpr (RM) {
+    if (rm.zp && blockIdx.x == 0)
+      for (int i = t; i < rm.zc16; i += NT) reinterpret_cast<uint4*>(rm.zp)[i] = uint4{0u, 0u, 0u, 0u};
+  }
   BnApply8 bn;
   bn.load(cg, gamma, mean, invstd, dgamma, dbeta, 1.f / (float)P);
   float s1[8] = {0};
@@ -663,7 +657,9 @@
     uint2 am[RU];
     Raw8<GDT> gr[RU];
     int64_t xoff[RU];
+    int64_t doff[RU];
     int pos0[RU], ix0[RU];
+    bool first[RU];
 #pragma unroll
     for (int v = 0; v < RU; ++v) {
       const int u = min(u0 + v * stride, units - 1);
@@ -680,6 +676,13 @@
       am[v] = *reinterpret_cast<const uint2*>(argmax + coff);
       gr[v].load(gm, coff);
       xoff[v] = ((int64_t)rowi * W + ix0[v]) * C + cg * 8;
+      if constexpr (RM) {
+        doff[v] = (rm.lead + (int64_t)rowi * rm.rowpx + ix0[v]) * C + cg * 8;
+        first[v] = rest == 0;
+      } else {
+        doff[v] = xoff[v];
+        first[v] = false;
+      }
 #pragma unroll
       for (int j = 0; j < KW; ++j) {
         const int64_t o = ix0[v] + j < W ? xoff[v] + (int64_t)j * C : xoff[v];
@@ -709,7 +712,15 @@
           }
           o4[q] = pk_bf16(g[0], g[1]);
         }
-        *reinterpret_cast<uint4*>(dx + xoff[v] + (int64_t)j * C) = uint4{o4[0], o4[1], o4[2], o4[3]};
+        *reinterpret_cast<uint4*>(dx + doff[v] + (int64_t)j * C) = uint4{o4[0], o4[1], o4[2], o4[3]};
+      }
+      if constexpr (RM) {
+        if (ix0[v] + KW >= W)
+          for (int px = W - ix0[v]; px < rm.rowpx - ix0[v]; ++px)
+            *reinterpret_cast<uint4*>(dx + doff[v] + (int64_t)px * C) = uint4{0u, 0u, 0u, 0u};
+        if (first[v])
+          for (int px = 0; px < rm.lead; ++px)
+            *reinterpret_cast<uint4*>(dx + (int64_t)px * C + cg * 8) = uint4{0u, 0u, 0u, 0u};
       }
     }
   }
@@ -969,7 +980,8 @@
 static int pool_bn_bwd_apply_launch(const void* gm, const uint8_t* argmax, const void* x, int32_t dtype, int32_t n,
                                     int32_t h, int32_t w, int32_t c, int32_t kh, int32_t kw, const float* gamma,
                                     const float* mean, const float* invstd, const float* dgamma, const float* dbeta,
-                                    void* dx, float* dbias, void* partial, hipStream_t s) {
+                                    void* dx, float* dbias, void* partial, hipStream_t s, const RowMap& rm) {
+  const bool mapped = rm.lead != 0 || rm.rowpx != w || rm.zp;
   const int rslots = NT / (c / 8);
   const int64_t P = (int64_t)n * h * w;
   const int64_t units = (int64_t)n * h * ((w + 7) / 8) * (c / 8);
@@ -981,7 +993,7 @@
     }
     return 0;
   };
-  if (kw % 8 == 0 && dtype == MIA_BF16 && units < (1ll << 31) &&
+  if (!mapped && kw % 8 == 0 && dtype == MIA_BF16 && units < (1ll << 31) &&
       ((reinterpret_cast<uintptr_t>(x) | reinterpret_cast<uintptr_t>(dx)) & 15) == 0) {
     const int nb = (int)std::max<int64_t>(1, std::min<int64_t>(cdiv(units, NT), CP_MAXBLK));
     pool_bn_bwd_apply_oct_kernel<GDT><<<nb, NT, 0, s>>>(gm, argmax, reinterpret_cast<const bf16*>(x), n, h, w, c, kh, kw,
@@ -995,11 +1007,24 @@
   if (kw >= 2 && kw <= 4 && dtype == MIA_BF16 && runs < (1ll << 31) && !per_pixel &&
       ((reinterpret_cast<uintptr_t>(x) | reinterpret_cast<uintptr_t>(dx)) & 15) == 0) {
     constexpr int RU = PB_RUNS;
-    const int nb = (int)std::max<int64_t>(1, std::min<int64_t>(cdiv(runs, (int64_t)NT * RU), PB_NB));
+    const int nb = pool_grid_cap((int)std::max<int64_t>(1, std::min<int64_t>(cdiv(runs, (int64_t)NT * RU), PB_NB)));
     const FastDiv dNR = make_fastdiv((int)cdiv(w, kw)), dH = make_fastdiv(h), dG = make_fastdiv(c / 8);
     float* part = dbias ? (float*)partial : nullptr;
     const bf16* xb = reinterpret_cast<const bf16*>(x);
     bf16* dxb = reinterpret_cast<bf16*>(dx);
+    if (mapped) {
+      MIA_CHECK_ARG(((int64_t)rm.lead + (int64_t)n * h * rm.rowpx) * c < (1ll << 40), "pool_bn_bwd_apply: row map size");
+      if (kw == 2)
+        pool_bn_bwd_apply_run_kernel<2, RU, GDT, true><<<nb, NT, 0, s>>>(gm, argmax, xb, n, h, w, c, kh, dNR, dH, dG, gamma,
+                                                                         mean, invstd, dgamma, dbeta, dxb, part, rm);
+      else if (kw == 3)
+        pool_bn_bwd_apply_run_kernel<3, RU, GDT, true><<<nb, NT, 0, s>>>(gm, argmax, xb, n, h, w, c, kh, dNR, dH, dG, gamma,
+                                                                         mean, invstd, dgamma, dbeta, dxb, part, rm);
+      else
+        pool_bn_bwd_apply_run_kernel<4, RU, GDT, true><<<nb, NT, 0, s>>>(gm, argmax, xb, n, h, w, c, kh, dNR, dH, dG, gamma,
+                                                                         mean, invstd, dgamma, dbeta, dxb, part, rm);
+      return finish("pool_bn_bwd_apply_run", nb);
+    }
     if (kw == 2)
       pool_bn_bwd_apply_run_kernel<2, RU, GDT><<<nb, NT, 0, s>>>(gm, argmax, xb, n, h, w, c, kh, dNR, dH, dG, gamma,
                                                                  mean, invstd, dgamma, dbeta, dxb, part);
@@ -1011,6 +1036,7 @@
                                                                  mean, invstd, dgamma, dbeta, dxb, part);
     return finish("pool_bn_bwd_apply_run", nb);
   }
+  MIA_CHECK_ARG(!mapped, "pool_bn_bwd_apply: a row map needs the run form (bf16, kw 2..4, 16-byte aligned x / dx)");
   const int nb = (int)std::max<int64_t>(1, std::min<int64_t>(cdiv(P, (int64_t)rslots * 8), CP_MAXBLK));
   pool_bn_bwd_apply_kernel<GDT><<<nb, NT, 0, s>>>(gm, argmax, x, dtype, n, h, w, c, kh, kw, make_fastdiv(w),
                                                   make_fastdiv(h), make_fastdiv(kw), make_fastdiv(kh), gamma, mean,
@@ -1018,11 +1044,15 @@
   return finish("pool_bn_bwd_apply", nb);
 }
 
-extern "C" int mia_pool_bn_relu_bwd_apply_ex(const void* gm, int32_t gm_dtype, const uint8_t* argmax, const void* x,
-                                             int32_t dtype, int32_t n, int32_t h, int32_t w, int32_t c, int32_t kh,
-                                             int32_t kw, const float* gamma, const float* mean, const float* invstd,
-                                             const float* dgamma, const float* dbeta, void* dx, float* dbias,
-                                             void* partial, mia_stream_t stream) {
+extern "C" int mia_pool_bn_relu_bwd_apply_rows(const void* gm, int32_t gm_dtype, const uint8_t* argmax, const void* x,
+                                               int32_t dtype, int32_t n, int32_t h, int32_t w, int32_t c, int32_t kh,
+                                               int32_t kw, const float* gamma, const float* mean, const float* invstd,
+                                               const float* dgamma, const float* dbeta, void* dx, int32_t lead,
+                                               int32_t row_pixels, void* zero_pixel, int32_t zc, float* dbias,
+                                               void* partial, mia_stream_t stream) {
+  MIA_CHECK_ARG(lead >= 0 && row_pixels >= w && zc >= 0 && zc % 8 == 0 && (zc == 0 || zero_pixel),
+                "pool_bn_bwd_apply: bad row map (lead %d, row_pixels %d, w %d, zc %d)", lead, row_pixels, w, zc);
+  MIA_CHECK_ARG(!zero_pixel || aligned16(zero_pixel), "pool_bn_bwd_apply: zero_pixel alignment");
   MIA_CHECK_ARG(gm && argmax && x && mean && invstd && dgamma && dbeta && dx, "pool_bn_bwd_apply: null pointer");
   MIA_CHECK_ARG(!dbias || partial, "pool_bn_bwd_apply: dbias needs the partial workspace");
   MIA_CHECK_ARG(c % 8 == 0 && c >= 8 && (NT % (c / 8)) == 0, "pool_bn_bwd_apply: channels");
@@ -1031,11 +1061,21 @@
   MIA_CHECK_ARG(gm_dtype == MIA_F32 || gm_dtype == MIA_BF16, "pool_bn_bwd_apply: gm dtype %d", gm_dtype);
   MIA_CHECK_ARG((reinterpret_cast<uintptr_t>(gm) & 15) == 0, "pool_bn_bwd_apply: gm alignment");
   hipStream_t s = as_stream(stream);
+  const RowMap rm{lead, row_pixels, zc ? zero_pixel : nullptr, zc / 8};
   if (gm_dtype == MIA_BF16)
     return pool_bn_bwd_apply_launch<MIA_BF16>(gm, argmax, x, dtype, n, h, w, c, kh, kw, gamma, mean, invstd, dgamma,
-                                              dbeta, dx, dbias, partial, s);
+                                              dbeta, dx, dbias, partial, s, rm);
   return pool_bn_bwd_apply_launch<MIA_F32>(gm, argmax, x, dtype, n, h, w, c, kh, kw, gamma, mean, invstd, dgamma, dbeta,
-                                           dx, dbias, partial, s);
+                                           dx, dbias, partial, s, rm);
+}
+
+extern "C" int mia_pool_bn_relu_bwd_apply_ex(const void* gm, int32_t gm_dtype, const uint8_t* argmax, const void* x,
+                                             int32_t dtype, int32_t n, int32_t h, int32_t w, int32_t c, int32_t kh,
+                                             int32_t kw, const float* gamma, const float* mean, const float* invstd,
+                                             const float* dgamma, const float* dbeta, void* dx, float* dbias,
+                                             void* partial, mia_stream_t stream) {
+  return mia_pool_bn_relu_bwd_apply_rows(gm, gm_dtype, argmax, x, dtype, n, h, w, c, kh, kw, gamma, mean, invstd, dgamma,
+                                         dbeta, dx, 0, w, nullptr, 0, dbias, partial, stream);
 }
 
 extern "C" int mia_pool_bn_relu_bwd_apply(const float* gm, const uint8_t* argmax, const void* x, int32_t dtype,
diff --git a/dl-sound-classification_amd/src/miaudio/kernels.py b/dl-sound-classification_amd/src/miaudio/kernels.py
--- a/dl-sound-classification_amd/src/miaudio/kernels.py
+++ b/dl-sound-classification_amd/src/miaudio/kernels.py
@@ -314,9 +314,18 @@
                                  dbeta.data_ptr(), L.ptr(dbias), ws.data_ptr(), _s()), "mia_bn_bwd_apply")
 
 
-def bn_relu_bwd_apply(dact, x, dx, P, C, gamma, bn: BNState, dgamma, dbeta, dbias=None):
+def bn_relu_bwd_apply(dact, x, dx, P, C, gamma, bn: BNState, dgamma, dbeta, dbias=None, rowmap=None):
     lib = L.load()
     ws = workspace(lib.mia_bn_partial_bytes(P, C), x.device, "bn")
+    if rowmap is not None:
+        w, lead, rowpx, zp = rowmap
+        assert dx.numel() == (lead + P // w * rowpx) * C
+        L.check(lib.mia_bn_relu_bwd_apply_rows(dact.data_ptr(), x.data_ptr(), dx.data_ptr(), L.dtype_code(x), P, C, w,
+                                               lead, rowpx, L.ptr(zp), 0 if zp is None else zp.numel(), L.ptr(gamma),
+                                               bn.scale.data_ptr(), bn.shift.data_ptr(), bn.mean.data_ptr(),
+                                               bn.invstd.data_ptr(), dgamma.data_ptr(), dbeta.data_ptr(),
+                                               L.ptr(dbias), ws.data_ptr(), _s()), "mia_bn_relu_bwd_apply_rows")
+        return
     L.check(lib.mia_bn_relu_bwd_apply(dact.data_ptr(), x.data_ptr(), dx.data_ptr(), L.dtype_code(x), P, C,
                                       L.ptr(gamma), bn.scale.data_ptr(), bn.shift.data_ptr(), bn.mean.data_ptr(),
                                       bn.invstd.data_ptr(), dgamma.data_ptr(), dbeta.data_ptr(), L.ptr(dbias),
@@ -341,9 +350,20 @@
     return gm, g[0], g[1]
 
 
-def pool_bn_relu_bwd_apply(gm, argmax, x, n, h, w, c, kh, kw, gamma, bn: BNState, dgamma, dbeta, dx, dbias=None):
+def pool_bn_relu_bwd_apply(gm, argmax, x, n, h, w, c, kh, kw, gamma, bn: BNState, dgamma, dbeta, dx, dbias=None,
+                           rowmap=None):
     lib = L.load()
     ws = workspace(lib.mia_bn_partial_bytes(n * h * w, c), x.device, "bn")
+    if rowmap is not None:
+        lead, rowpx, zp = rowmap
+        assert dx.numel() == (lead + n * h * rowpx) * c
+        L.check(lib.mia_pool_bn_relu_bwd_apply_rows(gm.data_ptr(), L.dtype_code(gm), argmax.data_ptr(), x.data_ptr(),
+                                                    L.dtype_code(x), n, h, w, c, kh, kw, L.ptr(gamma),
+                                                    bn.mean.data_ptr(), bn.invstd.data_ptr(), dgamma.data_ptr(),
+                                                    dbeta.data_ptr(), dx.data_ptr(), lead, rowpx, L.ptr(zp),
+                                                    0 if zp is None else zp.numel(), L.ptr(dbias), ws.data_ptr(),
+                                                    _s()), "mia_pool_bn_relu_bwd_apply_rows")
+        return
     L.check(lib.mia_pool_bn_relu_bwd_apply_ex(gm.data_ptr(), L.dtype_code(gm), argmax.data_ptr(), x.data_ptr(),
                                               L.dtype_code(x), n, h, w, c, kh, kw, L.ptr(gamma), bn.mean.data_ptr(),
                                               bn.invstd.data_ptr(), dgamma.data_ptr(), dbeta.data_ptr(),
@@ -592,23 +612,43 @@
 W2_DROPCOPY = os.environ.get("MIA_W2_DROPCOPY", "0") == "1"
 
 
+def w2_padcopy() -> bool:
+    return os.environ.get("MIA_W2_PADCOPY", "0") == "1"
+
+
+def w2_grad_buffer(rows: int, w: int, cout: int, a: torch.Tensor, cin: int):
+    if W2_SHIFT or w2_padcopy():
+        return None
+    P = rows * w
+    assert a.untyped_storage().nbytes() - a.storage_offset() * 2 >= (P + 1) * cin * 2, "a needs a pad pixel"
+    G = workspace((P + 1) * cout * 2, a.device, "w2shift")[: (P + 1) * cout * 2].view(torch.bfloat16)
+    pad = torch.empty(0, dtype=a.dtype, device=a.device).set_(a.untyped_storage(), a.storage_offset() + P * cin, (cin,))
+    return G, (1, w, pad)
+
+
 def trunk_bwd_w2(dy: torch.Tensor, a: torch.Tensor, rows: int, w: int, cout: int, cin: int, wpk: torch.Tensor,
-                 dw: torch.Tensor, dx: torch.Tensor, tag: str = "", wflip: torch.Tensor | None = None):
-    assert dy.dtype == torch.bfloat16 and a.dtype == torch.bfloat16 and dw.dtype == torch.float32
-    assert dy.numel() == rows * (w - 1) * cout and a.numel() == rows * w * cin and dw.numel() == cout * 2 * cin
+                 dw: torch.Tensor, dx: torch.Tensor, tag: str = "", wflip: torch.Tensor | None = None,
+                 G: torch.Tensor | None = None):
+    assert a.dtype == torch.bfloat16 and dw.dtype == torch.float32
+    assert a.numel() == rows * w * cin and dw.numel() == cout * 2 * cin
+    if G is None:
+        assert dy.dtype == torch.bfloat16 and dy.numel() == rows * (w - 1) * cout
     assert dx.numel() == rows * w * cin and dx.dtype == torch.bfloat16 and wpk.numel() == cout * 2 * cin
     P = rows * w
     if not W2_SHIFT and wflip is not None:
         assert a.untyped_storage().nbytes() - a.storage_offset() * 2 >= (P + 1) * cin * 2, "a needs a pad pixel"
-        G = workspace((P + 1) * cout * 2, dy.device, "w2shift")[: (P + 1) * cout * 2].view(torch.bfloat16)
-        L.check(L.load().mia_pad_w2(dy.data_ptr(), rows, w, cout, G.data_ptr(), a.data_ptr() + P * cin * 2, cin, _s()),
-                "mia_pad_w2")
+        if G is None:
+            G = workspace((P + 1) * cout * 2, dy.device, "w2shift")[: (P + 1) * cout * 2].view(torch.bfloat16)
+            L.check(L.load().mia_pad_w2(dy.data_ptr(), rows, w, cout, G.data_ptr(), a.data_ptr() + P * cin * 2, cin,
+                                        _s()), "mia_pad_w2")
+        assert G.dtype == torch.bfloat16 and G.numel() == (P + 1) * cout
         G1 = G[cout:]
         gemm(dense(G1, L.RC, P, cout), dense(a, L.RC, P, 2 * cin, ld=cin), epilogue(dw, 2 * cin), cout, 2 * cin, P,
              L.BF16, tag=f"{tag}.wgrad" if tag else None)
         gemm(dense(G, L.KC, P, 2 * cout, ld=cout), dense(wflip, L.KC, cin, 2 * cout), epilogue(dx, cin), P, cin,
              2 * cout, L.BF16, tag=f"{tag}.dgrad" if tag else None)
         return
+    assert G is None, "a laid-out G needs the pad form (wflip, not MIA_W2_SHIFT)"
     ash = workspace(P * 2 * cout * 2, dy.device, "w2shift")[: P * 2 * cout * 2].view(torch.bfloat16)
     L.check(L.load().mia_shift_pad_w2(dy.data_ptr(), rows, w, cout, ash.data_ptr(), _s()), "mia_shift_pad_w2")
     gemm(dense(ash, L.RC, P, 2 * cout), dense(a, L.RC, P, cin), epilogue(dw, cin), 2 * cout, cin, P, L.BF16,
diff --git a/dl-sound-classification_amd/src/miaudio/lib.py b/dl-sound-classification_amd/src/miaudio/lib.py
--- a/dl-sound-classification_amd/src/miaudio/lib.py
+++ b/dl-sound-classification_amd/src/miaudio/lib.py
@@ -97,6 +97,10 @@
                                          i32, vp, vp, vp, vp]),
     "mia_pool_bn_relu_bwd_apply_ex": (C.c_int, [vp, i32, vp, vp, i32, i32, i32, i32, i32, i32, i32, vp, vp, vp, vp, vp,
                                                 vp, vp, vp, vp]),
+    "mia_pool_bn_relu_bwd_apply_rows": (C.c_int, [vp, i32, vp, vp, i32, i32, i32, i32, i32, i32, i32, vp, vp, vp, vp,
+                                                  vp, vp, i32, i32, vp, i32, vp, vp, vp]),
+    "mia_bn_relu_bwd_apply_rows": (C.c_int, [vp, vp, vp, i32, i64, i32, i32, i32, i32, vp, i32, vp, vp, vp, vp, vp,
+                                             vp, vp, vp, vp, vp]),
     "mia_pool_fwd": (C.c_int, [vp, i32, i32, i32, i32, i32, i32, i32, vp, vp, vp, i32, vp, vp, vp]),
     "mia_pool_bwd_bn_relu_reduce": (C.c_int, [vp, i32, vp, vp, i32, i32, i32, i32, i32, i32, i32, vp, vp, vp,
                                               vp, vp, vp, vp, vp, vp]),
diff --git a/dl-sound-classification_amd/src/models/envnet_hip.py b/dl-sound-classification_amd/src/models/envnet_hip.py
--- a/dl-sound-classification_amd/src/models/envnet_hip.py
+++ b/dl-sound-classification_amd/src/models/envnet_hip.py
@@ -333,10 +333,16 @@
             gm, dgb, dbb = K.pool_bwd_gather(dpool, lay, ts["am"], ts["yb"], B, hb, wb, cout2, ph, pw, ts["bnb"],
                                              win=ts["win"])
             grads[pa + 6], grads[pa + 7] = dgb, dbb
-            dyb = torch.empty(Pb, cout2, dtype=tdt, device=dev)
             dbias_b = torch.empty(cout2, dtype=torch.float32, device=dev)
-            K.pool_bn_relu_bwd_apply(gm, ts["am"], ts["yb"], B, hb, wb, cout2, ph, pw, bns[3 + 2 * blk].weight,
-                                     ts["bnb"], dgb, dbb, dyb, dbias_b)
+            Gb = K.w2_grad_buffer(B * ha, wa, cout2, ts["act"], cin2) if ts["act"] is not None else None
+            if Gb is None:
+                dyb = torch.empty(Pb, cout2, dtype=tdt, device=dev)
+                K.pool_bn_relu_bwd_apply(gm, ts["am"], ts["yb"], B, hb, wb, cout2, ph, pw, bns[3 + 2 * blk].weight,
+                                         ts["bnb"], dgb, dbb, dyb, dbias_b)
+            else:
+                dyb = None
+                K.pool_bn_relu_bwd_apply(gm, ts["am"], ts["yb"], B, hb, wb, cout2, ph, pw, bns[3 + 2 * blk].weight,
+                                         ts["bnb"], dgb, dbb, Gb[0], dbias_b, rowmap=Gb[1])
             grads[pa + 5] = dbias_b
             Kb = kh2 * kw2 * cin2
             dWb = torch.empty(cout2, Kb, dtype=torch.float32, device=dev)
@@ -345,7 +351,7 @@
             red = None
             if ts["act"] is not None:
                 K.trunk_bwd_w2(dyb, ts["act"], B * ha, wa, cout2, cin2, wpk[pa + 4], dWb, da, wflip=wbk[(pa + 4, 1)],
-                               tag=f"t{blk}b")
+                               tag=f"t{blk}b", G=None if Gb is None else Gb[0])
             else:
                 K.gemm(K.dense(dyb, L.RC, Pb, cout2),
                        K.conv(ts["ya"], L.RC, B, ha, wa, cin2, hb, wb, kh2, kw2, pre=L.PRE_AFFINE_RELU,
@@ -373,9 +379,14 @@
             dWa = torch.empty(cout, Ka, dtype=torch.float32, device=dev)
             dense_w2 = ts["act"] is not None
             c3w = cin == 1 and cd == L.BF16 and kh == 8 and kw == 8 and cout == 32 and W % 4 == 0
+            Ga = K.w2_grad_buffer(B * H, W, cout, ts["inp"], cin) if dense_w2 else None
             if c3w and not C3_BNSEP:
                 K.conv3_wgrad_bn(ts["inp"], da, ts["ya"], da, dWa, dbias_a, B, H, W, bns[2 + 2 * blk].weight,
                                  ts["bna"], dga, dba, tag=f"t{blk}a.wgrad")
+            elif Ga is not None:
+                K.bn_relu_bwd_apply(da, ts["ya"], Ga[0], Pa, cout, bns[2 + 2 * blk].weight, ts["bna"], dga, dba,
+                                    dbias_a, rowmap=(wa, *Ga[1]))
+                dya = None
             else:
                 K.bn_relu_bwd_apply(da, ts["ya"], da, Pa, cout, bns[2 + 2 * blk].weight, ts["bna"], dga, dba,
                                     dbias_a)
@@ -384,7 +395,7 @@
             elif dense_w2:
                 dinp = torch.empty(B * H * W, cin, dtype=tdt, device=dev)
                 K.trunk_bwd_w2(dya, ts["inp"].reshape(B * H * W, cin), B * H, W, cout, cin, wpk[pa],
-                               dWa, dinp, tag=f"t{blk}a", wflip=wbk[(pa, 1)])
+                               dWa, dinp, tag=f"t{blk}a", wflip=wbk[(pa, 1)], G=None if Ga is None else Ga[0])
             elif c3w:
                 K.conv3_wgrad(ts["inp"], dya, dWa, B, H, W, tag=f"t{blk}a.wgrad")
             else:
diff --git a/include/miaudio_rowmap.h b/include/miaudio_rowmap.h
--- /dev/null
+++ b/include/miaudio_rowmap.h
@@ -0,0 +1,24 @@
+#ifndef MIAUDIO_ROWMAP_H
+#define MIAUDIO_ROWMAP_H
+#include "miaudio.h"
+
+#ifdef __cplusplus
+extern "C" {
+#endif
+
+int mia_pool_bn_relu_bwd_apply_rows(const void* gm, int32_t gm_dtype, const uint8_t* argmax, const void* x,
+                                    int32_t dtype, int32_t n, int32_t h, int32_t w, int32_t c, int32_t kh, int32_t kw,
+                                    const float* gamma, const float* mean, const float* invstd, const float* dgamma,
+                                    const float* dbeta, void* dx, int32_t lead, int32_t row_pixels, void* zero_pixel,
+                                    int32_t zc, float* dbias, void* partial, mia_stream_t stream);
+
+int mia_bn_relu_bwd_apply_rows(const void* dact, const void* x, void* dx, int32_t dtype, int64_t P, int32_t C,
+                               int32_t w, int32_t lead, int32_t row_pixels, void* zero_pixel, int32_t zc,
+                               const float* gamma, const float* scale, const float* shift, const float* mean,
+                               const float* invstd, const float* dgamma, const float* dbeta, float* dbias,
+                               void* partial, mia_stream_t stream);
+
+#ifdef __cplusplus
+}
+#endif
+#endif
```

New measurement: 16460 clips/s (median of 6 runs). 1.01x the previous value.
